# fims9000/SYNT_ISIC

Hardware: AMD Instinct MI355X
Metric: images/sec at 3x64x64 T=1000 (DDPM reverse-diffusion sampling) (higher is better)
Workload: dtype f32

## Files before the change

include/sisic.h:

```cpp
#ifndef SISIC_H
#define SISIC_H

#include <stdint.h>

#ifdef __cplusplus
extern "C" {
#endif

#define SISIC_ABI_VERSION 3

#define SISIC_OK 0
#define SISIC_EINVAL (-1)
#define SISIC_EHIP (-2)
#define SISIC_ESTATE (-3)
#define SISIC_ECANCEL (-4)

typedef struct sisic_ctx sisic_ctx;
typedef struct sisic_unet sisic_unet;
typedef struct sisic_resnet sisic_resnet;

int sisic_abi_version(void);
const char* sisic_last_error(void);

int sisic_create(int device_id, sisic_ctx** out);
int sisic_destroy(sisic_ctx* ctx);


typedef struct sisic_conv_args {
    const float* in0;
    const float* in1;
    int c0, c1;
    int B, Hin, Win;
    int upsample;
    int ksize;
    int stride;
    const float* w_packed;
    const float* bias;
    int Cout;
    const float* gn_scale;
    const float* gn_shift;
    int gn_silu;
    const float* chan_bias;
    int chan_bias_stride;
    const float* residual;
    int relu;
    float* out;
    int tile_cfg;
    const float* w_winograd;
    float* stats_out;
    const float* fin_gamma;
    const float* fin_beta;
    int fin_groups;
    float fin_eps;
    float* fin_scale;
    float* fin_shift;
    float* fin_mean_rstd;
} sisic_conv_args;

int sisic_conv_finalizes(const sisic_conv_args* args);

int sisic_conv_stats_slots(const sisic_conv_args* args);

int64_t sisic_conv_winograd_numel(int Cout, int Cin);
int sisic_conv_winograd_pack(sisic_ctx*, const float* w_oihw, int Cout, int Cin, float* u_packed, void* stream);

int64_t sisic_conv_s2_numel(int Cout, int Cin);
int sisic_conv_s2_pack(sisic_ctx*, const float* w_oihw, int Cout, int Cin, float* out, void* stream);

int64_t sisic_conv_packed_numel(int Cout, int Cin, int ksize);
int sisic_conv_pack_weights(sisic_ctx*, const float* w_oihw, int Cout, int Cin, int ksize,
                            float* w_packed, void* stream);
int sisic_conv2d(sisic_ctx*, const sisic_conv_args* args, void* stream);

int sisic_groupnorm_stats(sisic_ctx*, const float* in0, int c0, const float* in1, int c1,
                          int B, int HW, int groups, float eps,
                          const float* gamma, const float* beta,
                          float* scale, float* shift, void* stream);

int sisic_groupnorm_finalize(sisic_ctx*, const float* stats0, int c0, int slots0,
                             const float* stats1, int c1, int slots1,
                             int B, int HW, int groups, float eps,
                             const float* gamma, const float* beta,
                             float* scale, float* shift, void* stream);

int sisic_attention(sisic_ctx*, const float* qkv, float* out, int B, int C, int N, int head_dim,
                    void* stream);

int sisic_ddpm_step(sisic_ctx*, const float* eps, const float* x, const float* z, float* out,
                    int64_t n, float sqrt_beta_prod, float sqrt_alpha_prod, float c0, float c1,
                    float sigma, float clip, void* stream);

int sisic_denorm_u8(sisic_ctx*, const float* x, uint8_t* out, int B, int C, int H, int W, void* stream);
int sisic_denorm_u8_form(sisic_ctx*, const float* x, uint8_t* out, int B, int C, int H, int W, int form, void* stream);

typedef struct sisic_unet_config {
    int in_channels, out_channels;
    int layers_per_block;
    int n_blocks;
    int block_out_channels[8];
    int down_attn[8];
    int up_attn[8];
    int norm_groups;
    float norm_eps;
    int head_dim;
    int n_freqs;
    const float* freqs;
} sisic_unet_config;

int sisic_unet_create(sisic_ctx*, const sisic_unet_config* cfg, sisic_unet** out);
int sisic_unet_destroy(sisic_unet*);
int sisic_unet_num_tensors(const sisic_unet*);
const char* sisic_unet_tensor_name(const sisic_unet*, int index);
int sisic_unet_load(sisic_unet*, int n, const char* const* names, const float* const* host_ptrs,
                    const int64_t* numels);
int sisic_unet_set_latency_mode(sisic_unet*, int on);
int sisic_unet_set_graph_mode(sisic_unet*, int mode);
int64_t sisic_unet_graph_builds(const sisic_unet*);
int sisic_unet_forward(sisic_unet*, const float* sample, const int64_t* timesteps,
                       float* out, int B, int H, int W, void* stream);

int sisic_sample(sisic_unet*, float* x, int B, int H, int W, int T, const int64_t* timesteps,
                 const float* coef, float clip, const float* noise, float* traj, uint8_t* out_u8,
                 const volatile int* cancel, int* steps_done, void* stream);
int sisic_sample_frames(sisic_unet*, float* x, int B, int H, int W, int T, const int64_t* timesteps,
                        const float* coef, float clip, const float* noise, float* traj, const int* traj_row,
                        uint8_t* out_u8, const volatile int* cancel, int* steps_done, void* stream);

int sisic_noise_fill(sisic_ctx*, float* out, int B, int64_t n_per_image, const uint64_t* seeds, uint32_t step,
                     uint32_t tag, void* stream);
int sisic_noise_bits(sisic_ctx*, uint32_t* out, int B, int64_t n_per_image, const uint64_t* seeds, uint32_t step,
                     uint32_t tag, void* stream);
int sisic_ddpm_step_rng(sisic_ctx*, const float* eps, const float* x, float* out, int B, int64_t n_per_image,
                        const uint64_t* seeds_dev, uint32_t step, float sqrt_beta_prod, float sqrt_alpha_prod, float c0,
                        float c1, float sigma, float clip, void* stream);
int sisic_sample_frames_rng(sisic_unet*, float* x, int B, int H, int W, int T, const int64_t* timesteps,
                            const float* coef, float clip, const uint64_t* seeds, int step0, float* traj,
                            const int* traj_row, uint8_t* out_u8, const volatile int* cancel, int* steps_done,
                            void* stream);

int sisic_unet_train_begin(sisic_unet*);
int sisic_unet_train_end(sisic_unet*);
int sisic_add_noise(sisic_ctx*, const float* x0, const float* noise, const float* sqrt_alpha_prod,
                    const float* sqrt_one_minus_alpha_prod, float* out, int B, int64_t per_sample, void* stream);
int sisic_unet_train_forward(sisic_unet*, const float* sample, const int64_t* timesteps, float* out, int B, int H, int W,
                             void* stream);
int sisic_mse_loss(sisic_unet*, const float* pred, const float* target, int64_t n, float grad_scale, float* loss_dev,
                   float* dpred, void* stream);
int sisic_unet_backward(sisic_unet*, const float* dout, void* stream);
int sisic_unet_zero_grad(sisic_unet*, void* stream);
int sisic_unet_optimizer_step(sisic_unet*, double lr, double beta1, double beta2, double eps, float inv_scale, int* found_inf,
                              void* stream);
int sisic_unet_train_step(sisic_unet*, const float* images, const float* noise, const int64_t* timesteps,
                          const float* sqrt_alpha_prod, const float* sqrt_one_minus_alpha_prod, int B, int H, int W, double lr,
                          double beta1, double beta2, double eps, float loss_scale, float* loss_out, int* found_inf, void* stream);
int sisic_unet_read(sisic_unet*, int what, int index, float* host_out, int64_t numel);
int sisic_unet_write(sisic_unet*, int what, int index, const float* host_in, int64_t numel);
int64_t sisic_unet_train_steps(const sisic_unet*);

int sisic_conv2d_wgrad(sisic_ctx*, const sisic_conv_args* fwd_args, const float* dy, float* dw, void* stream);
int sisic_attention_bwd(sisic_ctx*, const float* qkv, const float* o, const float* dO, float* dqkv, int B, int C, int N,
                        int head_dim, void* stream);
int sisic_groupnorm_bwd(sisic_ctx*, const float* da, const float* x, int B, int C, int HW, int groups, float eps,
                        const float* gamma, const float* beta, int silu, float* dx_accum, float* dgamma, float* dbeta,
                        void* stream);

int sisic_resnet_create(sisic_ctx*, int num_classes, sisic_resnet** out);
int sisic_resnet_destroy(sisic_resnet*);
// ... 65 lines not shown
```

synt_isic_amd/_lib.py:

```python
from __future__ import annotations

import ctypes as C
import os
from typing import Optional

_LIB_PATH = os.environ.get("SISIC_LIB_PATH") or os.path.join(os.path.dirname(os.path.abspath(__file__)), "lib",
                                                             "libsisic_hip.so")
_lib: Optional[C.CDLL] = None

ABI_VERSION = 3

SISIC_OK = 0
SISIC_EINVAL = -1
SISIC_EHIP = -2
SISIC_ESTATE = -3
SISIC_ECANCEL = -4

c_float_p = C.POINTER(C.c_float)
c_int64_p = C.POINTER(C.c_int64)


class ConvArgs(C.Structure):
    _fields_ = [
        ("in0", C.c_void_p), ("in1", C.c_void_p),
        ("c0", C.c_int), ("c1", C.c_int),
        ("B", C.c_int), ("Hin", C.c_int), ("Win", C.c_int),
        ("upsample", C.c_int), ("ksize", C.c_int), ("stride", C.c_int),
        ("w_packed", C.c_void_p), ("bias", C.c_void_p), ("Cout", C.c_int),
        ("gn_scale", C.c_void_p), ("gn_shift", C.c_void_p), ("gn_silu", C.c_int),
        ("chan_bias", C.c_void_p), ("chan_bias_stride", C.c_int),
        ("residual", C.c_void_p), ("relu", C.c_int),
        ("out", C.c_void_p), ("tile_cfg", C.c_int),
        ("w_winograd", C.c_void_p),
        ("stats_out", C.c_void_p),
        ("fin_gamma", C.c_void_p), ("fin_beta", C.c_void_p), ("fin_groups", C.c_int), ("fin_eps", C.c_float),
        ("fin_scale", C.c_void_p), ("fin_shift", C.c_void_p), ("fin_mean_rstd", C.c_void_p),
    ]


class UNetConfigC(C.Structure):
    _fields_ = [
        ("in_channels", C.c_int), ("out_channels", C.c_int),
        ("layers_per_block", C.c_int), ("n_blocks", C.c_int),
        ("block_out_channels", C.c_int * 8),
        ("down_attn", C.c_int * 8), ("up_attn", C.c_int * 8),
        ("norm_groups", C.c_int), ("norm_eps", C.c_float), ("head_dim", C.c_int),
        ("n_freqs", C.c_int), ("freqs", c_float_p),
    ]


class InterventionJob(C.Structure):
    _fields_ = [("frame", C.c_int), ("mask", C.c_int), ("type", C.c_int), ("blur_kernel", C.c_int),
                ("noise_std", C.c_float)]


class AugmentParams(C.Structure):
    _fields_ = [("src", C.c_int32), ("crop_x", C.c_int32), ("crop_y", C.c_int32), ("crop_w", C.c_int32),
                ("crop_h", C.c_int32), ("hflip", C.c_int32), ("vflip", C.c_int32), ("order", C.c_int32 * 3),
                ("factor", C.c_float * 3), ("rotate", C.c_int32), ("rot", C.c_int32 * 6), ("reserved", C.c_int32 * 4)]


SIGNATURES = {
    "sisic_abi_version": (C.c_int, []),
    "sisic_last_error": (C.c_char_p, []),
    "sisic_create": (C.c_int, [C.c_int, C.POINTER(C.c_void_p)]),
    "sisic_destroy": (C.c_int, [C.c_void_p]),
    "sisic_conv_packed_numel": (C.c_int64, [C.c_int, C.c_int, C.c_int]),
    "sisic_conv_pack_weights": (C.c_int, [C.c_void_p, C.c_void_p, C.c_int, C.c_int, C.c_int, C.c_void_p, C.c_void_p]),
    "sisic_conv_winograd_numel": (C.c_int64, [C.c_int, C.c_int]),
    "sisic_conv_winograd_pack": (C.c_int, [C.c_void_p, C.c_void_p, C.c_int, C.c_int, C.c_void_p, C.c_void_p]),
    "sisic_conv_s2_numel": (C.c_int64, [C.c_int, C.c_int]),
    "sisic_conv_s2_pack": (C.c_int, [C.c_void_p, C.c_void_p, C.c_int, C.c_int, C.c_void_p, C.c_void_p]),
    "sisic_conv2d": (C.c_int, [C.c_void_p, C.POINTER(ConvArgs), C.c_void_p]),
    "sisic_conv_stats_slots": (C.c_int, [C.POINTER(ConvArgs)]),
    "sisic_conv_finalizes": (C.c_int, [C.POINTER(ConvArgs)]),
    "sisic_groupnorm_finalize": (C.c_int, [C.c_void_p, C.c_void_p, C.c_int, C.c_int, C.c_void_p, C.c_int, C.c_int,
                                           C.c_int, C.c_int, C.c_int, C.c_float, C.c_void_p, C.c_void_p, C.c_void_p,
                                           C.c_void_p, C.c_void_p]),
    "sisic_groupnorm_stats": (C.c_int, [C.c_void_p, C.c_void_p, C.c_int, C.c_void_p, C.c_int, C.c_int, C.c_int,
                                        C.c_int, C.c_float, C.c_void_p, C.c_void_p, C.c_void_p, C.c_void_p,
                                        C.c_void_p]),
    "sisic_attention": (C.c_int, [C.c_void_p, C.c_void_p, C.c_void_p, C.c_int, C.c_int, C.c_int, C.c_int, C.c_void_p]),
    "sisic_ddpm_step": (C.c_int, [C.c_void_p, C.c_void_p, C.c_void_p, C.c_void_p, C.c_void_p, C.c_int64,
                                  C.c_float, C.c_float, C.c_float, C.c_float, C.c_float, C.c_float, C.c_void_p]),
    "sisic_denorm_u8": (C.c_int, [C.c_void_p, C.c_void_p, C.c_void_p, C.c_int, C.c_int, C.c_int, C.c_int, C.c_void_p]),
    "sisic_denorm_u8_form": (C.c_int, [C.c_void_p, C.c_void_p, C.c_void_p, C.c_int, C.c_int, C.c_int, C.c_int, C.c_int,
                                       C.c_void_p]),
    "sisic_unet_create": (C.c_int, [C.c_void_p, C.POINTER(UNetConfigC), C.POINTER(C.c_void_p)]),
    "sisic_unet_destroy": (C.c_int, [C.c_void_p]),
    "sisic_unet_num_tensors": (C.c_int, [C.c_void_p]),
    "sisic_unet_tensor_name": (C.c_char_p, [C.c_void_p, C.c_int]),
    "sisic_unet_load": (C.c_int, [C.c_void_p, C.c_int, C.POINTER(C.c_char_p), C.POINTER(C.c_void_p), c_int64_p]),
    "sisic_unet_set_latency_mode": (C.c_int, [C.c_void_p, C.c_int]),
    "sisic_unet_set_graph_mode": (C.c_int, [C.c_void_p, C.c_int]),
    "sisic_unet_graph_builds": (C.c_int64, [C.c_void_p]),
    "sisic_unet_forward": (C.c_int, [C.c_void_p, C.c_void_p, c_int64_p, C.c_void_p, C.c_int, C.c_int, C.c_int,
                                     C.c_void_p]),
    "sisic_sample": (C.c_int, [C.c_void_p, C.c_void_p, C.c_int, C.c_int, C.c_int, C.c_int, c_int64_p, c_float_p,
                               C.c_float, C.c_void_p, C.c_void_p, C.c_void_p, C.POINTER(C.c_int), C.POINTER(C.c_int),
                               C.c_void_p]),
    "sisic_sample_frames": (C.c_int, [C.c_void_p, C.c_void_p, C.c_int, C.c_int, C.c_int, C.c_int, c_int64_p, c_float_p,
                                      C.c_float, C.c_void_p, C.c_void_p, C.POINTER(C.c_int), C.c_void_p, C.POINTER(C.c_int),
                                      C.POINTER(C.c_int), C.c_void_p]),
    "sisic_noise_fill": (C.c_int, [C.c_void_p, C.c_void_p, C.c_int, C.c_int64, C.POINTER(C.c_uint64), C.c_uint32,
                                   C.c_uint32, C.c_void_p]),
    "sisic_noise_bits": (C.c_int, [C.c_void_p, C.c_void_p, C.c_int, C.c_int64, C.POINTER(C.c_uint64), C.c_uint32,
                                   C.c_uint32, C.c_void_p]),
    "sisic_ddpm_step_rng": (C.c_int, [C.c_void_p, C.c_void_p, C.c_void_p, C.c_void_p, C.c_int, C.c_int64, C.c_void_p,
                                      C.c_uint32, C.c_float, C.c_float, C.c_float, C.c_float, C.c_float, C.c_float,
                                      C.c_void_p]),
    "sisic_sample_frames_rng": (C.c_int, [C.c_void_p, C.c_void_p, C.c_int, C.c_int, C.c_int, C.c_int, c_int64_p, c_float_p,
                                          C.c_float, C.POINTER(C.c_uint64), C.c_int, C.c_void_p, C.POINTER(C.c_int),
                                          C.c_void_p, C.POINTER(C.c_int), C.POINTER(C.c_int), C.c_void_p]),
    "sisic_unet_train_begin": (C.c_int, [C.c_void_p]),
    "sisic_unet_train_end": (C.c_int, [C.c_void_p]),
    "sisic_add_noise": (C.c_int, [C.c_void_p, C.c_void_p, C.c_void_p, C.c_void_p, C.c_void_p, C.c_void_p, C.c_int,
                                  C.c_int64, C.c_void_p]),
    "sisic_unet_train_forward": (C.c_int, [C.c_void_p, C.c_void_p, c_int64_p, C.c_void_p, C.c_int, C.c_int, C.c_int,
                                           C.c_void_p]),
    "sisic_mse_loss": (C.c_int, [C.c_void_p, C.c_void_p, C.c_void_p, C.c_int64, C.c_float, C.c_void_p, C.c_void_p,
                                 C.c_void_p]),
    "sisic_unet_backward": (C.c_int, [C.c_void_p, C.c_void_p, C.c_void_p]),
    "sisic_unet_zero_grad": (C.c_int, [C.c_void_p, C.c_void_p]),
    "sisic_unet_optimizer_step": (C.c_int, [C.c_void_p, C.c_double, C.c_double, C.c_double, C.c_double, C.c_float,
                                            C.POINTER(C.c_int), C.c_void_p]),
    "sisic_unet_train_step": (C.c_int, [C.c_void_p, C.c_void_p, C.c_void_p, c_int64_p, c_float_p, c_float_p, C.c_int,
                                        C.c_int, C.c_int, C.c_double, C.c_double, C.c_double, C.c_double, C.c_float,
                                        C.POINTER(C.c_float), C.POINTER(C.c_int), C.c_void_p]),
    "sisic_unet_read": (C.c_int, [C.c_void_p, C.c_int, C.c_int, c_float_p, C.c_int64]),
    "sisic_unet_write": (C.c_int, [C.c_void_p, C.c_int, C.c_int, c_float_p, C.c_int64]),
    "sisic_unet_train_steps": (C.c_int64, [C.c_void_p]),
    "sisic_conv2d_wgrad": (C.c_int, [C.c_void_p, C.POINTER(ConvArgs), C.c_void_p, C.c_void_p, C.c_void_p]),
    "sisic_attention_bwd": (C.c_int, [C.c_void_p, C.c_void_p, C.c_void_p, C.c_void_p, C.c_void_p, C.c_int, C.c_int, C.c_int,
                                      C.c_int, C.c_void_p]),
    "sisic_groupnorm_bwd": (C.c_int, [C.c_void_p, C.c_void_p, C.c_void_p, C.c_int, C.c_int, C.c_int, C.c_int, C.c_float,
                                      C.c_void_p, C.c_void_p, C.c_int, C.c_void_p, C.c_void_p, C.c_void_p, C.c_void_p]),
    "sisic_resnet_create": (C.c_int, [C.c_void_p, C.c_int, C.POINTER(C.c_void_p)]),
    "sisic_resnet_destroy": (C.c_int, [C.c_void_p]),
    "sisic_resnet_num_tensors": (C.c_int, [C.c_void_p]),
    "sisic_resnet_tensor_name": (C.c_char_p, [C.c_void_p, C.c_int]),
    "sisic_resnet_load": (C.c_int, [C.c_void_p, C.c_int, C.POINTER(C.c_char_p), C.POINTER(C.c_void_p), c_int64_p]),
    "sisic_resnet_randomize": (C.c_int, [C.c_void_p, C.c_uint64, C.c_uint32, C.c_float, C.c_void_p]),
    "sisic_resnet_restore": (C.c_int, [C.c_void_p, C.c_void_p]),
    "sisic_resnet_forward": (C.c_int, [C.c_void_p, C.c_void_p, C.c_void_p, C.c_int, C.c_int, C.c_int, C.c_int,
                                       C.c_void_p]),
    "sisic_resnet_stem": (C.c_int, [C.c_void_p, C.c_void_p, C.c_void_p, C.c_int, C.c_int, C.c_int, C.c_int, C.c_void_p]),
    "sisic_resnet_input_gradient": (C.c_int, [C.c_void_p, C.c_void_p, C.c_int, C.c_int, C.c_int, C.c_int, C.c_void_p,
                                              C.c_void_p, C.c_void_p]),
    "sisic_resnet_gradcam": (C.c_int, [C.c_void_p, C.c_void_p, C.c_int, C.c_int, C.c_int, C.c_int, C.c_void_p,
                                       C.c_void_p, C.c_void_p]),
    "sisic_resnet_workspace_bytes": (C.c_int64, [C.c_void_p]),
    "sisic_unet_workspace_bytes": (C.c_int64, [C.c_void_p]),
    "sisic_class_scores": (C.c_int, [C.c_void_p, C.c_void_p, C.c_int, C.c_int, C.c_int, C.c_void_p, C.c_void_p,
                                     C.c_void_p]),
    "sisic_mask_patches": (C.c_int, [C.c_void_p, C.c_void_p, C.c_void_p, C.c_void_p, C.c_int, C.c_int, C.c_int,
                                     C.c_int, C.c_int, C.c_void_p]),
    "sisic_intervene": (C.c_int, [C.c_void_p, C.c_void_p, C.c_int, C.c_void_p, C.c_int, C.c_int, C.c_int, C.c_int, C.c_int,
                                  C.POINTER(InterventionJob), C.POINTER(C.c_uint64), C.c_void_p, C.c_void_p, C.c_void_p,
                                  C.c_void_p, C.c_void_p]),
    "sisic_cfi_metrics": (C.c_int, [C.c_void_p, C.c_void_p, C.c_int, C.c_void_p, C.c_int, C.c_int, C.POINTER(C.c_int),
                                    C.c_void_p, C.c_void_p]),
# ... 48 lines not shown
```

synt_isic_amd/csrc/api.cpp:

```cpp
#include <cstring>

#include "common.h"

namespace sisic {

static thread_local char g_err[1024] = "";

void set_error(const char* fmt, ...) {
    va_list ap;
    va_start(ap, fmt);
    vsnprintf(g_err, sizeof(g_err), fmt, ap);
    va_end(ap);
}

static hipEvent_t take_event(sisic_ctx* ctx) {
    if (!ctx->event_pool.empty()) {
        hipEvent_t e = ctx->event_pool.back();
        ctx->event_pool.pop_back();
        return e;
    }
    hipEvent_t e = nullptr;
    if (hipEventCreate(&e) != hipSuccess) return nullptr;
    return e;
}

ProfileScope::ProfileScope(sisic_ctx* c, hipStream_t s, int kind, double bytes, double flops, double flops_exec, int kind2)
    : ctx(c), stream(s) {
    if (!c || !c->profiling) return;
    ev.start = take_event(c);
    ev.stop = take_event(c);
    ev.kind = kind;
    ev.kind2 = kind2;
    if (!ev.start || !ev.stop) return;
    for (int k : {kind, kind2}) {
        if (k < 0) continue;
        c->prof[k].bytes += bytes;
        c->prof[k].flops += flops;
        c->prof[k].flops_exec += (flops_exec < 0.0) ? flops : flops_exec;
        c->prof[k].launches += 1;
    }
    (void)hipEventRecord(ev.start, s);
    active = true;
}

ProfileScope::~ProfileScope() {
    if (!active) return;
    (void)hipEventRecord(ev.stop, stream);
    ctx->pending.push_back(ev);
}

int profile_collect(sisic_ctx* ctx) {
    for (auto& ev : ctx->pending) {
        SISIC_HIP(hipEventSynchronize(ev.stop));
        float ms = 0.f;
        SISIC_HIP(hipEventElapsedTime(&ms, ev.start, ev.stop));
        ctx->prof[ev.kind].ms += ms;
        if (ev.kind2 >= 0) ctx->prof[ev.kind2].ms += ms;
        ctx->event_pool.push_back(ev.start);
        ctx->event_pool.push_back(ev.stop);
    }
    ctx->pending.clear();
    return SISIC_OK;
}

}

using namespace sisic;

extern "C" {

int sisic_abi_version(void) { return SISIC_ABI_VERSION; }

const char* sisic_last_error(void) { return sisic::g_err; }

int sisic_create(int device_id, sisic_ctx** out) {
    SISIC_REQUIRE(out != nullptr, "sisic_create: out is NULL");
    *out = nullptr;
    int n = 0;
    SISIC_HIP(hipGetDeviceCount(&n));
    SISIC_REQUIRE(device_id >= 0 && device_id < n, "sisic_create: device %d of %d", device_id, n);
    SISIC_HIP(hipSetDevice(device_id));
    hipDeviceProp_t prop;
    SISIC_HIP(hipGetDeviceProperties(&prop, device_id));
    SISIC_REQUIRE(std::strncmp(prop.gcnArchName, "gfx950", 6) == 0,
                  "sisic_create: device %d is %s; this library is built for gfx950 (MI355X) only", device_id,
                  prop.gcnArchName);
    auto* ctx = new sisic_ctx();
    ctx->device = device_id;
    ctx->num_cus = prop.multiProcessorCount;
    *out = ctx;
    return SISIC_OK;
}

int sisic_destroy(sisic_ctx* ctx) {
    if (!ctx) return SISIC_OK;
    (void)profile_collect(ctx);
    for (auto e : ctx->event_pool) (void)hipEventDestroy(e);
    for (auto& kv : ctx->splitk)
        if (kv.second.p) (void)hipFree(kv.second.p);
    for (auto& it : ctx->bf3_items) {
        if (it.fill_done) (void)hipEventDestroy(it.fill_done);
        if (it.tab) (void)hipFree(it.tab);
    }
    delete ctx;
    return SISIC_OK;
}

int64_t sisic_conv_packed_numel(int Cout, int Cin, int ksize) {
    if (Cout <= 0 || Cin <= 0 || (ksize != 1 && ksize != 3 && ksize != 7)) return -1;
    return conv_packed_floats(Cout, Cin, ksize);
}

int sisic_conv_pack_weights(sisic_ctx* ctx, const float* w, int Cout, int Cin, int ksize, float* packed, void* stream) {
    SISIC_REQUIRE(ctx && w && packed && Cout > 0 && Cin > 0, "conv_pack_weights: bad arguments");
    return launch_conv_pack(ctx, w, Cout, Cin, ksize, packed, static_cast<hipStream_t>(stream));
}

int64_t sisic_conv_s2_numel(int Cout, int Cin) {
    if (Cout <= 0 || Cin <= 0) return -1;
    return conv_s2_packed_floats(Cout, Cin);
}

int sisic_conv_s2_pack(sisic_ctx* ctx, const float* w, int Cout, int Cin, float* out, void* stream) {
    SISIC_REQUIRE(ctx && w && out && Cout > 0 && Cin > 0, "conv_s2_pack: bad arguments");
    return launch_conv_s2_pack(ctx, w, Cout, Cin, out, static_cast<hipStream_t>(stream));
}

int64_t sisic_conv_winograd_numel(int Cout, int Cin) {
    if (Cout <= 0 || Cin <= 0) return -1;
    return winograd_packed_numel(Cout, Cin);
}

int sisic_conv_winograd_pack(sisic_ctx* ctx, const float* w, int Cout, int Cin, float* packed, void* stream) {
    SISIC_REQUIRE(ctx && w && packed && Cout > 0 && Cin > 0, "conv_winograd_pack: bad arguments");
    return launch_winograd_pack(ctx, w, Cout, Cin, packed, static_cast<hipStream_t>(stream));
}

int sisic_conv2d(sisic_ctx* ctx, const sisic_conv_args* args, void* stream) {
    SISIC_REQUIRE(ctx && args, "conv2d: null argument");
    return launch_conv2d(ctx, *args, static_cast<hipStream_t>(stream));
}

int sisic_conv_stats_slots(const sisic_conv_args* args) { return args ? conv_stats_slots(*args) : 0; }
int sisic_conv_finalizes(const sisic_conv_args* args) { return args && conv_finalizes(*args) ? 1 : 0; }

int sisic_groupnorm_finalize(sisic_ctx* ctx, const float* stats0, int c0, int slots0, const float* stats1, int c1,
                             int slots1, int B, int HW, int groups, float eps, const float* gamma, const float* beta,
                             float* scale, float* shift, void* stream) {
    SISIC_REQUIRE(ctx, "groupnorm_finalize: null context");
    return launch_gn_finalize(ctx, stats0, c0, slots0, stats1, c1, slots1, B, HW, groups, eps, gamma, beta, scale,
                              shift, static_cast<hipStream_t>(stream));
}

int sisic_groupnorm_stats(sisic_ctx* ctx, const float* in0, int c0, const float* in1, int c1, int B, int HW,
                          int groups, float eps, const float* gamma, const float* beta, float* scale, float* shift,
                          void* stream) {
    SISIC_REQUIRE(ctx, "groupnorm_stats: null context");
    return launch_gn_stats(ctx, in0, c0, in1, c1, B, HW, groups, eps, gamma, beta, scale, shift,
                           static_cast<hipStream_t>(stream));
}

int sisic_attention(sisic_ctx* ctx, const float* qkv, float* out, int B, int C, int N, int head_dim, void* stream) {
    SISIC_REQUIRE(ctx, "attention: null context");
    return launch_attention(ctx, qkv, out, B, C, N, head_dim, static_cast<hipStream_t>(stream));
}

int sisic_ddpm_step(sisic_ctx* ctx, const float* eps, const float* x, const float* z, float* out, int64_t n,
                    float sqrt_beta_prod, float sqrt_alpha_prod, float c0, float c1, float sigma, float clip,
                    void* stream) {
    SISIC_REQUIRE(ctx, "ddpm_step: null context");
    return launch_ddpm_step(ctx, eps, x, z, out, n, sqrt_beta_prod, sqrt_alpha_prod, c0, c1, sigma, clip,
                            static_cast<hipStream_t>(stream));
}

int sisic_noise_fill(sisic_ctx* ctx, float* out, int B, int64_t n_per_image, const uint64_t* seeds, uint32_t step,
                     uint32_t tag, void* stream) {
    SISIC_REQUIRE(ctx, "noise_fill: null context");
    return launch_noise_fill(ctx, out, B, n_per_image, seeds, step, tag, false, static_cast<hipStream_t>(stream));
}

int sisic_noise_bits(sisic_ctx* ctx, uint32_t* out, int B, int64_t n_per_image, const uint64_t* seeds, uint32_t step,
                     uint32_t tag, void* stream) {
    SISIC_REQUIRE(ctx, "noise_bits: null context");
    return launch_noise_fill(ctx, out, B, n_per_image, seeds, step, tag, true, static_cast<hipStream_t>(stream));
}

int sisic_ddpm_step_rng(sisic_ctx* ctx, const float* eps, const float* x, float* out, int B, int64_t n_per_image,
                        const uint64_t* seeds_dev, uint32_t step, float sqrt_beta_prod, float sqrt_alpha_prod, float c0,
                        float c1, float sigma, float clip, void* stream) {
    SISIC_REQUIRE(ctx && B > 0 && n_per_image > 0, "ddpm_step_rng: null context or empty batch");
    return launch_ddpm_step_rng(ctx, eps, x, out, (int64_t)B * n_per_image, n_per_image, seeds_dev, step, sqrt_beta_prod,
                                sqrt_alpha_prod, c0, c1, sigma, clip, static_cast<hipStream_t>(stream));
}

int sisic_denorm_u8(sisic_ctx* ctx, const float* x, uint8_t* out, int B, int C, int H, int W, void* stream) {
    SISIC_REQUIRE(ctx, "denorm_u8: null context");
    return launch_denorm_u8(ctx, x, out, B, C, H, W, static_cast<hipStream_t>(stream));
}

int sisic_denorm_u8_form(sisic_ctx* ctx, const float* x, uint8_t* out, int B, int C, int H, int W, int form, void* stream) {
    SISIC_REQUIRE(ctx, "denorm_u8_form: null context");
    return launch_denorm_u8(ctx, x, out, B, C, H, W, static_cast<hipStream_t>(stream), form);
}

int sisic_intervene(sisic_ctx* ctx, const float* frames, int F, const uint8_t* masks, int M, int C, int H, int W, int J,
                    const sisic_intervention_job* jobs, const uint64_t* seeds, const int32_t* src_index, float* out,
                    float* intervention_out, float* stats, void* stream) {
    SISIC_REQUIRE(ctx, "intervene: null context");
    return launch_intervene(ctx, frames, F, masks, M, C, H, W, J, jobs, seeds, src_index, out, intervention_out, stats,
                            static_cast<hipStream_t>(stream));
}

int sisic_cfi_metrics(sisic_ctx* ctx, const float* logits_orig, int F, const float* logits_mod, int J, int n_classes,
                      const int* job_frame, float* rows, void* stream) {
    SISIC_REQUIRE(ctx, "cfi_metrics: null context");
    return launch_cfi_metrics(ctx, logits_orig, F, logits_mod, J, n_classes, job_frame, rows, static_cast<hipStream_t>(stream));
}

int sisic_resample_diffs(sisic_ctx* ctx, const double* top, int n_top, const double* bottom, int n_bottom, uint64_t seed,
                         int n_bootstrap, int n_permutations, double* boot_out, double* perm_out, void* stream) {
    SISIC_REQUIRE(ctx, "resample_diffs: null context");
    return launch_resample_diffs(ctx, top, n_top, bottom, n_bottom, seed, n_bootstrap, n_permutations, boot_out, perm_out,
                                 static_cast<hipStream_t>(stream));
}

int sisic_augment(sisic_ctx* ctx, const uint8_t* dataset, int N, int H, int W, const sisic_augment_params* params_dev, int B,
                  int32_t* gray_mean_scratch, float* out, void* stream) {
    SISIC_REQUIRE(ctx, "augment: null context");
    return launch_augment(ctx, dataset, N, H, W, params_dev, B, gray_mean_scratch, out, false, static_cast<hipStream_t>(stream));
}

int sisic_augment_u8(sisic_ctx* ctx, const uint8_t* dataset, int N, int H, int W, const sisic_augment_params* params_dev,
                     int B, int32_t* gray_mean_scratch, uint8_t* out_hwc, void* stream) {
    SISIC_REQUIRE(ctx, "augment_u8: null context");
    return launch_augment(ctx, dataset, N, H, W, params_dev, B, gray_mean_scratch, out_hwc, true, static_cast<hipStream_t>(stream));
}
// ... 28 lines not shown
```

synt_isic_amd/csrc/common.h:

```cpp
#pragma once

#include <hip/hip_runtime.h>

#include <atomic>
#include <cstdarg>
#include <cstdint>
#include <cstdio>
#include <string>
#include <map>
#include <mutex>
#include <vector>

#include "../../include/sisic.h"

namespace sisic {

void set_error(const char* fmt, ...);

#define SISIC_HIP(call)                                                                   \
    do {                                                                                  \
        hipError_t _e = (call);                                                           \
        if (_e != hipSuccess) {                                                           \
            ::sisic::set_error("%s failed: %s (%s:%d)", #call, hipGetErrorString(_e),     \
                               __FILE__, __LINE__);                                       \
// ... 9 lines not shown
        }                                        \
    } while (0)

#define SISIC_TRY(expr)             \
    do {                            \
        int _rc = (expr);           \
        if (_rc != SISIC_OK) return _rc; \
    } while (0)

enum ProfileKind { PK_CONV3 = 0, PK_CONV1 = 1, PK_GN = 2, PK_ATTN = 3, PK_DDPM = 4, PK_OTHER = 5, PK_WINO_MAIN = 6, PK_WINO_BF3 = 7, PK_COUNT = 8 };

struct ProfileSlot {
    double ms = 0, bytes = 0, flops = 0, flops_exec = 0;
    int64_t launches = 0;
};

struct PendingEvent {
    hipEvent_t start, stop;
    int kind;
    int kind2;
};

}

struct sisic_ctx {
    int device = 0;
    int num_cus = 0;
    bool profiling = false;
    sisic::ProfileSlot prof[sisic::PK_COUNT];
    std::vector<sisic::PendingEvent> pending;
    std::vector<hipEvent_t> event_pool;
    struct SplitK { float* p = nullptr; size_t floats = 0; };
    std::map<hipStream_t, SplitK> splitk;
    std::mutex splitk_mutex;
    struct Bf3Items { int key[9]; unsigned* tab = nullptr; hipStream_t fill_stream = nullptr; hipEvent_t fill_done = nullptr; };
    std::vector<Bf3Items> bf3_items;
    std::mutex bf3_items_mutex;
    std::atomic<uint64_t> scratch_generation{0};
};

namespace sisic {

struct ProfileScope {
    sisic_ctx* ctx;
    hipStream_t stream;
    PendingEvent ev{};
    bool active = false;
    ProfileScope(sisic_ctx* c, hipStream_t s, int kind, double bytes, double flops, double flops_exec = -1.0, int kind2 = -1);
    ~ProfileScope();
};

int profile_collect(sisic_ctx* ctx);

inline int ensure_dynamic_lds(sisic_ctx* ctx, const void* kern, int bytes, std::atomic<uint64_t>& done) {
    const uint64_t bit = uint64_t(1) << (ctx->device & 63);
    if (done.load(std::memory_order_acquire) & bit) return SISIC_OK;
    SISIC_HIP(hipFuncSetAttribute(kern, hipFuncAttributeMaxDynamicSharedMemorySize, bytes));
    done.fetch_or(bit, std::memory_order_release);
    return SISIC_OK;
}

inline int cdiv(int a, int b) { return (a + b - 1) / b; }
inline int wino_latency_ksplit(int Cout, int Cin, int Hout, int Wout) {
    const int co_t = Cout > 64 ? 128 : 64;
    const int per_image = cdiv(Hout, 8) * cdiv(Wout, 16) * cdiv(Cout, co_t);
    const int nchunks = cdiv(Cin, 8);
    int k = 1;
    while (per_image * k < 256 && k < 8 && nchunks % (2 * k) == 0) k *= 2;
    return k;
}
inline int wino_latency_segments(int Hout, int Wout) { return cdiv(Hout * Wout, 1024); }
inline int64_t cdiv64(int64_t a, int64_t b) { return (a + b - 1) / b; }
inline int round_up(int a, int b) { return cdiv(a, b) * b; }

constexpr int CONV_CO_TILE = 64;
inline int conv_ci_chunk(int ksize) { return ksize == 1 ? 32 : (ksize == 3 ? 16 : 4); }
inline int conv_cin_pad(int cin, int ksize) { return round_up(cin, conv_ci_chunk(ksize)); }
inline int conv_cout_pad(int cout) { return round_up(cout, CONV_CO_TILE); }
inline int64_t conv_packed_floats(int cout, int cin, int ksize) {
    const int64_t first = (int64_t)conv_cin_pad(cin, ksize) * ksize * ksize * conv_cout_pad(cout);
    return ksize == 1 ? 3 * first + first / 2 : first;
}

int launch_conv2d(sisic_ctx*, const sisic_conv_args& a, hipStream_t s);
int launch_conv_smallcout(sisic_ctx*, const sisic_conv_args& a, hipStream_t s);
int launch_score_head_bwd(sisic_ctx*, const float* logits, const float* fc_w, const float* act, float* g, int B, int C,
                          int HW, int n_classes, int target, hipStream_t s);
int launch_relu_bwd(sisic_ctx*, const float* dy, const float* y, float* out, int64_t n, hipStream_t s);
int launch_scatter_add_even(sisic_ctx*, float* dst, const float* src, int planes, int H, int W, hipStream_t s);
int launch_maxpool_bwd(sisic_ctx*, const float* dm, const float* xin, float* dx, int planes, int H, int W, hipStream_t s);
int launch_stem_bwd(sisic_ctx*, const float* g, const float* w_oihw, float* dp, int B, int CO, int OH, int OW, int H, int W,
                    hipStream_t s);
int launch_preprocess_bwd(sisic_ctx*, const float* dp, const float* x, float* dx, int B, int H, int W, int OH, int OW,
                          hipStream_t s);
int launch_add_relu(sisic_ctx*, const float* y, const float* identity, float* out, int64_t n, hipStream_t s);
int launch_gradcam(sisic_ctx*, const float* y, const float* outp, const float* fc_w, const float* bias, float* cam, int B, int C,
                   int h, int w, int S, int target, hipStream_t s);
int conv_stats_slots(const sisic_conv_args& a);
bool conv_finalizes(const sisic_conv_args& a);
bool conv_pointwise_applicable(const sisic_conv_args& a);
int conv_pointwise_stats_slots(const sisic_conv_args& a);
int launch_conv_pointwise(sisic_ctx*, const sisic_conv_args& a, hipStream_t s);
bool conv_pointwise_bf3_applicable(const sisic_conv_args& a);
int launch_conv_pointwise_bf3(sisic_ctx*, const sisic_conv_args& a, hipStream_t s);
bool conv_s2_bf3_applicable(const sisic_conv_args& a);
int conv_s2_bf3_stats_slots(const sisic_conv_args& a);
int launch_conv_s2_bf3(sisic_ctx*, const sisic_conv_args& a, hipStream_t s);
int64_t conv_s2_packed_floats(int Cout, int Cin);
int launch_conv_s2_pack(sisic_ctx*, const float* w, int Cout, int Cin, float* out, hipStream_t s);
int launch_gn_finalize(sisic_ctx*, const float* st0, int c0, int slots0, const float* st1, int c1, int slots1, int B,
                       int HW, int groups, float eps, const float* gamma, const float* beta, float* scale, float* shift,
                       hipStream_t s, float* mean_rstd = nullptr);
int launch_conv_winograd(sisic_ctx*, const sisic_conv_args& a, const float* u_packed, int cfg, hipStream_t s);
int launch_winograd_pack(sisic_ctx*, const float* w, int Cout, int Cin, float* packed, hipStream_t s);
int64_t winograd_packed_numel(int Cout, int Cin);
inline int64_t winograd_first_floats(int Cout, int Cin) { return (int64_t)round_up(Cin, 16) * 16 * conv_cout_pad(Cout); }
int launch_conv_pack(sisic_ctx*, const float* w, int Cout, int Cin, int k, float* packed, hipStream_t s);
int launch_gn_stats(sisic_ctx*, const float* in0, int c0, const float* in1, int c1, int B, int HW, int groups,
                    float eps, const float* gamma, const float* beta, float* scale, float* shift, hipStream_t s,
                    float* mean_rstd = nullptr);
int launch_attention(sisic_ctx*, const float* qkv, float* out, int B, int C, int N, int head_dim, hipStream_t s);
int launch_ddpm_step(sisic_ctx*, const float* eps, const float* x, const float* z, float* out, int64_t n,
                     float sb, float sa, float c0, float c1, float sigma, float clip, hipStream_t s);
size_t loop_state_bytes();
int launch_loop_select_row(sisic_ctx*, const float* table, int R, const void* state, float* out, hipStream_t s);
int launch_loop_advance(sisic_ctx*, void* state, hipStream_t s);
int launch_ddpm_step_indexed(sisic_ctx*, const float* eps, float* x, int64_t n, const void* state, const float* coef,
                             const int* zrow, float clip, hipStream_t s);
int launch_ddpm_step_rng(sisic_ctx*, const float* eps, const float* x, float* out, int64_t n, int64_t n_per_image,
                         const uint64_t* seeds_dev, uint32_t step, float sb, float sa, float c0, float c1, float sigma,
                         float clip, hipStream_t s);
int launch_ddpm_step_indexed_rng(sisic_ctx*, const float* eps, float* x, int64_t n, int64_t n_per_image, const void* state,
                                 const float* coef, const uint64_t* seeds_dev, float clip, hipStream_t s);
int launch_noise_fill(sisic_ctx*, void* out, int B, int64_t n_per_image, const uint64_t* seeds_host, uint32_t step,
                      uint32_t tag, bool bits, hipStream_t s);
int launch_denorm_u8(sisic_ctx*, const float* x, uint8_t* out, int B, int C, int H, int W, hipStream_t s, int form = 0);
int launch_temb_mlp(sisic_ctx*, const float* t_vals, int B, const float* freqs, int n_freqs, const float* w1t,
                    const float* b1, const float* w2t, const float* b2, int hidden, float* temb_act, hipStream_t s,
                    float* save_emb = nullptr, float* save_h1 = nullptr, float* save_t2 = nullptr);
int launch_linear_t(sisic_ctx*, const float* x, int B, int K, const float* wt, const float* bias, int R,
                    float* out, hipStream_t s);
int launch_transpose2d(sisic_ctx*, const float* in, int rows, int cols, float* out, int out_ld, int out_col0,
                       hipStream_t s);
int launch_preprocess(sisic_ctx*, const float* x, float* out, int B, int H, int W, int OH, int OW, hipStream_t s);
int launch_maxpool(sisic_ctx*, const float* x, float* out, int B, int C, int H, int W, hipStream_t s);
int launch_avgpool_fc(sisic_ctx*, const float* x, const float* w, const float* bias, float* out, int B, int C, int HW,
                      int n_out, hipStream_t s);
int launch_class_scores(sisic_ctx*, const float* logits, int B, int n, int target, float* prob, float* logscore,
                        hipStream_t s);
int launch_mask_patches(sisic_ctx*, const float* image, const uint8_t* masks, float* out, int S, int C, int H, int W,
                        int patch, hipStream_t s);

int launch_intervene(sisic_ctx*, const float* frames, int F, const uint8_t* masks, int M, int C, int H, int W, int J,
                     const sisic_intervention_job* jobs, const uint64_t* seeds, const int32_t* src_index, float* out,
                     float* intervention_out, float* stats, hipStream_t s);
int launch_cfi_metrics(sisic_ctx*, const float* logits_orig, int F, const float* logits_mod, int J, int n,
                       const int* job_frame, float* rows, hipStream_t s);
int launch_resample_diffs(sisic_ctx*, const double* top, int n_top, const double* bottom, int n_bottom, uint64_t seed,
                          int n_bootstrap, int n_permutations, double* boot_out, double* perm_out, hipStream_t s);
int launch_randomize_weight(sisic_ctx*, float* raw, float* raw_t, const double* sc, int cout, int cin, int k, uint64_t seed,
                            uint32_t trial, uint32_t tag, float strength, hipStream_t s);

int launch_augment(sisic_ctx*, const uint8_t* dataset, int N, int H, int W, const sisic_augment_params* params_dev, int B,
                   int32_t* gray_mean_scratch, void* out, bool u8, hipStream_t s);

}
```

synt_isic_amd/csrc/conv_mfma.hip:

```cpp
#include <cstdlib>
#include <type_traits>

#include "common.h"
#include "pack_device.h"

namespace sisic {

typedef float f32x16 __attribute__((ext_vector_type(16)));

struct ConvParams {
    const float* in0;
    const float* in1;
    int c0, c1;
    int B, Hin, Win;
    int Hc, Wc;
    int Hout, Wout;
    int ups;
    int zero_insert;
    const float* w;
    int cout_pad;
    const float* bias;
    int Cout;
    const float* gn_scale;
    const float* gn_shift;
// ... 322 lines not shown
                psum[m][r] += pv ? v : 0.0f;
            }
        }
    }

    if (p.stats) {
        const float cnt = half_wave_sum((float)__builtin_popcount(pvmask));
        const float inv = 1.0f / fmaxf(cnt, 1.0f);
        const int slots = p.tiles_x * p.tiles_y * WN, slot = (ty * p.tiles_x + tx) * WN + wn;
#pragma unroll
        for (int m = 0; m < MT; ++m) {
#pragma unroll
            for (int r = 0; r < 16; ++r) {
                const int co = co0 + wm * MT * 32 + m * 32 + (r & 3) + 8 * (r >> 2) + 4 * half;
                const float s1 = half_wave_sum(psum[m][r]);
                const float mean = s1 * inv;
                float q = 0.0f;
#pragma unroll
                for (int n = 0; n < NT; ++n) {
                    const float d = acc[m][n][r] - mean;
                    q += ((pvmask >> n) & 1u) ? d * d : 0.0f;
                }
                q = half_wave_sum(q);
                if (l31 == 0 && co < p.Cout)
                    reinterpret_cast<float4*>(p.stats)[((size_t)b * p.Cout + co) * slots + slot] = make_float4(cnt, s1, q, 0.0f);
            }
        }
    }
}


__global__ void conv_pack_kernel(const float* __restrict__ w, int Cout, int Cin, int KK, int cin_pad, int cout_pad,
                                 float* __restrict__ out) {
    const size_t first = (size_t)cin_pad * KK * cout_pad;
    const size_t total = KK == 1 ? 3 * first + first / 2 : first;
    for (size_t i = (size_t)blockIdx.x * blockDim.x + threadIdx.x; i < total; i += (size_t)gridDim.x * blockDim.x) {
        conv_pack_elem(i, w, Cout, Cin, KK, cin_pad, cout_pad, out);
    }
}

template <int KS, int STRIDE, int MT, int NT, int WM, int WN, int TW, int CIC, int OCC = 2, int KSP = 1>
static int launch_cfg(sisic_ctx* ctx, ConvParams& p, hipStream_t s) {
    using G = ConvGeom<KS, STRIDE, MT, NT, WM, WN, TW, CIC, KSP>;
    p.tiles_x = cdiv(p.Wout, TW);
    p.tiles_y = cdiv(p.Hout, G::TH);
    p.n_co_tiles = p.cout_pad / G::CO_TILE;
    p.nchunks = cdiv(p.c0 + p.c1, CIC);
    const int64_t nwg = (int64_t)p.B * p.tiles_x * p.tiles_y * p.n_co_tiles;
    SISIC_REQUIRE(nwg > 0 && nwg < (int64_t(1) << 31), "conv2d: grid of %lld workgroups unsupported", (long long)nwg);
    p.nwg = (int)nwg;
    if (p.slots_query) {
        *p.slots_query = p.tiles_x * p.tiles_y * WN;
        return SISIC_OK;
    }
    if constexpr (KS == 1 && STRIDE == 1 && TW == G::PIX && G::EPT % 4 == 0) {
        const bool aligned = ((reinterpret_cast<uintptr_t>(p.in0) | reinterpret_cast<uintptr_t>(p.in1)) & 15) == 0;
        if (p.Wc % 4 == 0 && aligned) {
            auto kern4 = conv_mfma_kernel<KS, STRIDE, MT, NT, WM, WN, TW, CIC, OCC, KSP, true>;
            static std::atomic<uint64_t> lds_opt_in4{0};
            SISIC_TRY(ensure_dynamic_lds(ctx, reinterpret_cast<const void*>(kern4), (int)G::LDS_BYTES, lds_opt_in4));
            hipLaunchKernelGGL(kern4, dim3(p.nwg), dim3(G::NTHR), G::LDS_BYTES, s, p);
            SISIC_HIP(hipGetLastError());
            return SISIC_OK;
        }
    }
    auto kern = conv_mfma_kernel<KS, STRIDE, MT, NT, WM, WN, TW, CIC, OCC, KSP>;
    static std::atomic<uint64_t> lds_opt_in{0};
    SISIC_TRY(ensure_dynamic_lds(ctx, reinterpret_cast<const void*>(kern), (int)G::LDS_BYTES, lds_opt_in));
    hipLaunchKernelGGL(kern, dim3(p.nwg), dim3(G::NTHR), G::LDS_BYTES, s, p);
    SISIC_HIP(hipGetLastError());
    return SISIC_OK;
}

int launch_conv_pack(sisic_ctx*, const float* w, int Cout, int Cin, int k, float* packed, hipStream_t s) {
    SISIC_REQUIRE(k == 1 || k == 3 || k == 7, "conv_pack: ksize %d unsupported", k);
    const int cin_pad = conv_cin_pad(Cin, k), cout_pad = conv_cout_pad(Cout);
    const size_t total = (size_t)cin_pad * k * k * cout_pad;
    const int blocks = (int)std::min<size_t>((total * (k == 1 ? 4 : 1) + 255) / 256, 4096);
    hipLaunchKernelGGL(conv_pack_kernel, dim3(blocks), dim3(256), 0, s, w, Cout, Cin, k * k, cin_pad, cout_pad, packed);
    SISIC_HIP(hipGetLastError());
    return SISIC_OK;
}

static int dispatch_conv2d(sisic_ctx* ctx, const sisic_conv_args& a, hipStream_t s, int* slots_query);

static int winograd_cfg(const sisic_conv_args& a) {
    if (!(a.ksize == 3 && a.stride == 1 && a.w_winograd != nullptr && a.Cout > 4) || a.upsample == 2) return 0;
    if ((a.tile_cfg >= 60 && a.tile_cfg <= 74) || a.tile_cfg == 78 || a.tile_cfg == 79 || (a.tile_cfg >= 90 && a.tile_cfg <= 92)) return a.tile_cfg;
    if (a.tile_cfg != 0) return 0;
    const int Hout = a.Hin << (a.upsample ? 1 : 0), Wout = a.Win << (a.upsample ? 1 : 0);
    const bool fits32 = 16.0 * std::max(a.c0, a.c1) * a.Hin * a.Win < 4294967296.0;
    if (!fits32) return 0;
    if (Hout >= 12 && Wout >= 12) {
        static const bool wide_on = [] { const char* e = std::getenv("SISIC_WINO_WIDE"); return !e || std::atoi(e) != 0; }();
        static const bool bf3_on = [] { const char* e = std::getenv("SISIC_WINO_BF16X3"); return !e || std::atoi(e) != 0; }();
        const int th = (Hout + 15) / 16 * 16, tw = (Wout + 15) / 16 * 16;
        if (bf3_on && a.Cout % 64 == 0 && 4 * Hout * Wout >= 3 * th * tw && a.c0 + a.c1 >= 16 &&
            a.c0 + a.c1 <= 2048 &&
            4.0 * a.Cout * Hout * Wout < 2147483648.0)
            return 74;
        if (wide_on && !a.upsample) return a.Cout > 64 ? 68 : 69;
        return 66;
    }
    const int Cin = a.c0 + a.c1;
    static const bool ksplit_on = [] { const char* e = std::getenv("SISIC_KSPLIT"); return !e || std::atoi(e) != 0; }();
    if (ksplit_on && Hout <= 8 && Wout <= 8 && Hout >= 5 && Wout >= 5 && Cin >= 128 && Cin % 32 == 0 && a.Cout >= 128) {
        static const bool wide_on = [] { const char* e = std::getenv("SISIC_WINO_WIDE"); return !e || std::atoi(e) != 0; }();
        static const bool bf3_on = [] { const char* e = std::getenv("SISIC_WINO_BF16X3"); return !e || std::atoi(e) != 0; }();
        if (bf3_on && !a.upsample && a.Cout % 64 == 0 && Cin <= 512) return 92;
        return (wide_on && !a.upsample) ? 91 : 90;
    }
    return 0;
}
static bool winograd_selected(const sisic_conv_args& a) { return winograd_cfg(a) != 0; }

int conv_stats_slots(const sisic_conv_args& a) {
    if (const int cfg = winograd_cfg(a)) {
        if (cfg >= 90 && cfg <= 92) return 1;
        const int Hout = a.Hin << (a.upsample ? 1 : 0), Wout = a.Win << (a.upsample ? 1 : 0);
        if ((cfg == 78 || cfg == 79) && wino_latency_ksplit(a.Cout, a.c0 + a.c1, Hout, Wout) > 1) return wino_latency_segments(Hout, Wout);
        if ((cfg >= 68 && cfg <= 73) || cfg == 78 || cfg == 79) return ((Hout + 7) / 8) * ((Wout + 15) / 16);
        const int edge = (cfg == 61 || cfg == 63 || cfg == 65 || cfg == 67) ? 8 : 16;
        return ((Hout + edge - 1) / edge) * ((Wout + edge - 1) / edge);
    }
    int slots = 0;
    sisic_conv_args q = a;
    q.stats_out = nullptr;
    if (dispatch_conv2d(nullptr, q, nullptr, &slots) != SISIC_OK) return 0;
    return slots;
}

bool conv_finalizes(const sisic_conv_args& a) {
    if (!a.fin_gamma || a.fin_groups <= 0) return false;
    const int cfg = winograd_cfg(a);
    const int Hout = a.Hin << (a.upsample ? 1 : 0), Wout = a.Win << (a.upsample ? 1 : 0);
    if (a.Cout % a.fin_groups != 0 || a.Cout / a.fin_groups != 8) return false;
    if (cfg == 74) return !a.upsample && Hout <= 16 && Wout <= 16 && a.Cout % 64 == 0;
    if (cfg < 90 || cfg > 92) return false;
    if (Hout * Wout != 64 || a.Cout % 16 != 0) return false;
    return ((reinterpret_cast<uintptr_t>(a.residual) | reinterpret_cast<uintptr_t>(a.out) | reinterpret_cast<uintptr_t>(a.stats_out)) & 15) == 0;
}

int launch_conv2d(sisic_ctx* ctx, const sisic_conv_args& a, hipStream_t s) { return dispatch_conv2d(ctx, a, s, nullptr); }

static int dispatch_conv2d(sisic_ctx* ctx, const sisic_conv_args& a, hipStream_t s, int* slots_query) {
    SISIC_REQUIRE(a.in0 && a.w_packed && a.out, "conv2d: null tensor");
    SISIC_REQUIRE(a.B > 0 && a.Hin > 0 && a.Win > 0 && a.c0 > 0 && a.c1 >= 0 && a.Cout > 0, "conv2d: bad shape");
    SISIC_REQUIRE((a.c1 == 0) == (a.in1 == nullptr), "conv2d: in1/c1 mismatch");
    SISIC_REQUIRE(a.ksize == 1 || a.ksize == 3 || a.ksize == 7, "conv2d: ksize %d unsupported", a.ksize);
    SISIC_REQUIRE(a.stride == 1 || a.stride == 2, "conv2d: stride %d unsupported", a.stride);
    SISIC_REQUIRE(a.ksize != 7 || a.stride == 2, "conv2d: 7x7 is built for stride 2 only (the ResNet stem)");
    SISIC_REQUIRE(!(a.upsample && a.stride != 1), "conv2d: upsample with stride");
    SISIC_REQUIRE((a.gn_scale == nullptr) == (a.gn_shift == nullptr), "conv2d: gn_scale/gn_shift mismatch");

    ConvParams p{};
    p.in0 = a.in0; p.in1 = a.in1; p.c0 = a.c0; p.c1 = a.c1;
    p.B = a.B; p.Hin = a.Hin; p.Win = a.Win;
    p.ups = a.upsample ? 1 : 0;
    p.zero_insert = a.upsample == 2 ? 1 : 0;
    p.Hc = a.Hin << p.ups; p.Wc = a.Win << p.ups;
    const int pad = a.ksize / 2;
    p.Hout = (p.Hc + 2 * pad - a.ksize) / a.stride + 1;
    p.Wout = (p.Wc + 2 * pad - a.ksize) / a.stride + 1;
    p.w = a.w_packed; p.cout_pad = conv_cout_pad(a.Cout);
    p.bias = a.bias; p.Cout = a.Cout;
    p.gn_scale = a.gn_scale; p.gn_shift = a.gn_shift; p.gn_silu = a.gn_silu;
    p.chan_bias = a.chan_bias; p.chan_bias_stride = a.chan_bias_stride; p.residual = a.residual; p.relu = a.relu; p.out = a.out;
    p.stats = a.stats_out; p.slots_query = slots_query;

    const int Cin = a.c0 + a.c1;
    const double kk = double(a.ksize) * a.ksize;
    const double out_elems = double(a.B) * a.Cout * p.Hout * p.Wout;
    const double bytes = 4.0 * (double(a.B) * Cin * a.Hin * a.Win + out_elems) + 4.0 * (Cin * a.Cout * kk + a.Cout) +
                         (a.residual ? 4.0 * out_elems : 0.0);
    const double flops = 2.0 * out_elems * Cin * kk;
    int cfg = a.tile_cfg;
    const bool use_wino = winograd_selected(a);
    SISIC_REQUIRE(a.stats_out == nullptr || conv_stats_slots(a) > 0,
                  "conv2d: stats_out given but sisic_conv_stats_slots() is 0 for these arguments");
    const bool wino_ups9 = use_wino && a.upsample && !a.gn_scale && winograd_cfg(a) == 66;
    ProfileScope prof(slots_query ? nullptr : ctx, s, a.ksize == 1 ? PK_CONV1 : PK_CONV3, bytes, flops,
                      use_wino ? flops * (wino_ups9 ? 9.0 : 16.0) / 36.0 : flops,
                      (use_wino && winograd_cfg(a) == 74) ? PK_WINO_BF3 :
                      (use_wino && !wino_ups9 && (winograd_cfg(a) == 66 || (winograd_cfg(a) >= 68 && winograd_cfg(a) <= 73) || winograd_cfg(a) == 78 || winograd_cfg(a) == 79)) ? PK_WINO_MAIN : -1);

    if (a.ksize == 3 && a.stride == 1 && !a.upsample && a.Cout <= 4 && (cfg == 0 || (cfg >= 50 && cfg <= 52))) {
        if (slots_query) return SISIC_OK;
        return launch_conv_smallcout(ctx, a, s);
    }
    if (use_wino) {
        SISIC_REQUIRE(!slots_query, "conv2d: internal: slot query on the Winograd path");
        return launch_conv_winograd(ctx, a, a.w_winograd, winograd_cfg(a), s);
    }
    SISIC_REQUIRE((cfg < 60 || cfg > 74) && cfg != 78 && cfg != 79 && (cfg < 90 || cfg > 92), "conv2d: tile_cfg %d needs w_winograd, ksize 3 and stride 1", cfg);
    if (a.ksize == 7) {
        if (cfg == 0) cfg = 41;
        if (cfg == 41) return launch_cfg<7, 2, 2, 1, 1, 4, 32, 2>(ctx, p, s);
        if (cfg == 42) return launch_cfg<7, 2, 2, 1, 1, 4, 32, 4>(ctx, p, s);
    } else if (a.ksize == 1 && a.stride == 2) {
        if (cfg == 0) cfg = p.Wout >= 24 ? 31 : (p.Wout >= 12 ? 32 : 33);
        switch (cfg) {
            case 31: return launch_cfg<1, 2, 2, 1, 1, 4, 32, 16>(ctx, p, s);
            case 32: return launch_cfg<1, 2, 2, 1, 1, 4, 16, 16>(ctx, p, s);
            case 33: return launch_cfg<1, 2, 1, 1, 2, 2, 8, 16>(ctx, p, s);
        }
    } else if (a.ksize == 1) {
        p.Hin = 1; p.Win = a.Hin * a.Win; p.Hc = 1; p.Wc = p.Win; p.Hout = 1; p.Wout = p.Win; p.ups = 0;
        SISIC_REQUIRE(!a.upsample, "conv2d: 1x1 with upsample");
        static const bool pw_on = [] { const char* e = std::getenv("SISIC_POINTWISE"); return !e || std::atoi(e) != 0; }();
        static const bool pwb_on = [] { const char* e = std::getenv("SISIC_POINTWISE_BF16X3"); return !e || std::atoi(e) != 0; }();
        if ((cfg == 0 && pwb_on && conv_pointwise_bf3_applicable(a)) || (cfg >= 28 && cfg <= 30) || cfg == 34 || cfg == 35) {
            if (slots_query) { *slots_query = conv_pointwise_stats_slots(a); return SISIC_OK; }
            return launch_conv_pointwise_bf3(ctx, a, s);
        }
        if ((cfg == 0 && pw_on && conv_pointwise_applicable(a)) || cfg == 20) {
            if (slots_query) { *slots_query = conv_pointwise_stats_slots(a); return SISIC_OK; }
            return launch_conv_pointwise(ctx, a, s);
        }
        if (cfg == 0) cfg = (p.Wout <= 64) ? 22 : (p.Wout <= 256 ? 25 : 24);
        switch (cfg) {
            case 21: return launch_cfg<1, 1, 2, 2, 1, 4, 256, 16>(ctx, p, s);
            case 22: return launch_cfg<1, 1, 1, 1, 2, 2, 64, 16>(ctx, p, s);
            case 23: return launch_cfg<1, 1, 2, 1, 1, 4, 128, 16>(ctx, p, s);
            case 24: return launch_cfg<1, 1, 1, 2, 2, 4, 256, 32, 4>(ctx, p, s);
            case 25: return launch_cfg<1, 1, 1, 1, 2, 4, 128, 32, 4>(ctx, p, s);
            case 26: return launch_cfg<1, 1, 1, 2, 2, 4, 256, 16, 4>(ctx, p, s);
            case 27: return launch_cfg<1, 1, 1, 1, 2, 4, 128, 16, 4>(ctx, p, s);
        }
    } else if (a.stride == 1) {
        if (cfg == 0) cfg = p.Wout >= 24 ? 8 : (p.Wout >= 12 ? 9 : 16);
        switch (cfg) {
            case 1: return launch_cfg<3, 1, 2, 2, 1, 4, 64, 8>(ctx, p, s);
            case 2: return launch_cfg<3, 1, 2, 2, 1, 4, 32, 8>(ctx, p, s);
            case 3: return launch_cfg<3, 1, 2, 2, 1, 4, 16, 8>(ctx, p, s);
            case 4: return launch_cfg<3, 1, 1, 1, 2, 2, 8, 8>(ctx, p, s);
            case 16: return launch_cfg<3, 1, 1, 1, 2, 2, 8, 16, 2, 2>(ctx, p, s);
            case 17: return launch_cfg<3, 1, 1, 1, 2, 2, 8, 8, 2, 2>(ctx, p, s);
            case 5: return launch_cfg<3, 1, 2, 1, 1, 4, 16, 8>(ctx, p, s);
            case 6: return launch_cfg<3, 1, 2, 1, 1, 4, 64, 8>(ctx, p, s);
            case 7: return launch_cfg<3, 1, 2, 1, 1, 4, 32, 8>(ctx, p, s);
            case 8: return launch_cfg<3, 1, 1, 2, 2, 4, 32, 8, 4>(ctx, p, s);
            case 9: return launch_cfg<3, 1, 1, 2, 2, 4, 16, 8, 4>(ctx, p, s);
            case 10: return launch_cfg<3, 1, 1, 2, 2, 4, 32, 8, 2>(ctx, p, s);
            case 14: return launch_cfg<3, 1, 1, 1, 2, 4, 16, 8, 4>(ctx, p, s);
            case 15: return launch_cfg<3, 1, 1, 1, 2, 4, 8, 8, 4>(ctx, p, s);
        }
    } else {
        static const bool s2b_on = [] { const char* e = std::getenv("SISIC_S2_BF16X3"); return !e || std::atoi(e) != 0; }();
        if ((cfg == 0 && s2b_on && conv_s2_bf3_applicable(a)) || cfg == 36) {
            if (slots_query) { *slots_query = conv_s2_bf3_applicable(a) ? conv_s2_bf3_stats_slots(a) : 0; return SISIC_OK; }
            return launch_conv_s2_bf3(ctx, a, s);
        }
        if (cfg == 0) cfg = p.Wout >= 24 ? 11 : (p.Wout >= 12 ? 12 : 18);
        switch (cfg) {
            case 11: return launch_cfg<3, 2, 2, 1, 1, 4, 32, 8>(ctx, p, s);
            case 12: return launch_cfg<3, 2, 2, 1, 1, 4, 16, 8>(ctx, p, s);
            case 13: return launch_cfg<3, 2, 1, 1, 2, 2, 8, 8>(ctx, p, s);
            case 18: return launch_cfg<3, 2, 1, 1, 2, 2, 8, 16, 2, 2>(ctx, p, s);
            case 19: return launch_cfg<3, 2, 1, 1, 2, 2, 8, 8, 2, 2>(ctx, p, s);
        }
    }
    set_error("conv2d: tile_cfg %d invalid for ksize %d stride %d", cfg, a.ksize, a.stride);
    return SISIC_EINVAL;
}

}
```

synt_isic_amd/csrc/conv_pointwise_bf3.hip:

```cpp
#include <cstdlib>
#include <type_traits>

#include "common.h"

namespace sisic {

typedef float pwb_f32x16 __attribute__((ext_vector_type(16)));
typedef short pwb_bf16x8 __attribute__((ext_vector_type(8)));
typedef unsigned pwb_u4 __attribute__((ext_vector_type(4)));
typedef unsigned pwb_u2 __attribute__((ext_vector_type(2)));
typedef float pwb_f2 __attribute__((ext_vector_type(2)));
typedef float pwb_f4 __attribute__((ext_vector_type(4)));

struct PwbParams {
    const float* in0;
    const float* in1;
    int c0, c1, B, HW;
    const float* wb;
    int n_co64;
    const float* bias;
    int Cout;
    const float* gn_scale;
    const float* gn_shift;
    const float* chan_bias;
    int chan_bias_stride;
    const float* residual;
    int relu;
    float* out;
    float* stats;
    int n_px, n_co_items, nitems, nwg, nchunks;
};

constexpr int PWB_WAVES = 4;

__device__ __forceinline__ float pwb_half_wave_sum(float v) {
    v += __int_as_float(__builtin_amdgcn_update_dpp(0, __float_as_int(v), 0xB1, 0xf, 0xf, true));
    v += __int_as_float(__builtin_amdgcn_update_dpp(0, __float_as_int(v), 0x4E, 0xf, 0xf, true));
    v += __int_as_float(__builtin_amdgcn_update_dpp(0, __float_as_int(v), 0x141, 0xf, 0xf, true));
    v += __int_as_float(__builtin_amdgcn_update_dpp(0, __float_as_int(v), 0x140, 0xf, 0xf, true));
    return v + __shfl_xor(v, 16);
}
__device__ __forceinline__ float pwb_row16_sum(float v) {
    v += __int_as_float(__builtin_amdgcn_update_dpp(0, __float_as_int(v), 0xB1, 0xf, 0xf, true));
    v += __int_as_float(__builtin_amdgcn_update_dpp(0, __float_as_int(v), 0x4E, 0xf, 0xf, true));
    v += __int_as_float(__builtin_amdgcn_update_dpp(0, __float_as_int(v), 0x141, 0xf, 0xf, true));
    v += __int_as_float(__builtin_amdgcn_update_dpp(0, __float_as_int(v), 0x140, 0xf, 0xf, true));
    return v;
}
__device__ __forceinline__ float pwb_silu(float v) { return v * __builtin_amdgcn_rcpf(1.0f + __expf(-v)); }

template <int PRO, int NB>
__global__ void __launch_bounds__(64 * PWB_WAVES, 4) conv_pwb_kernel(const PwbParams p) {
    extern __shared__ __attribute__((aligned(16))) float smem[];
    int wg;
    {
        const int L = blockIdx.x, nwg = p.nwg;
        const int xcd = L & 7, slot = L >> 3, q = nwg >> 3, r = nwg & 7;
        wg = (xcd < r ? xcd * (q + 1) : r * (q + 1) + (xcd - r) * q) + slot;
    }
    const int tid = threadIdx.x, lane = tid & 63;
    const int wave_u = __builtin_amdgcn_readfirstlane(tid >> 6);
    const int item = wg * PWB_WAVES + wave_u;
    if (item >= p.nitems) return;
    const int half = lane >> 5, l31 = lane & 31;
    int co_i = item % p.n_co_items;
    const int t = item / p.n_co_items;
    int px_t = t % p.n_px, b = t / p.n_px;
    asm volatile("" : "+s"(co_i), "+s"(px_t), "+s"(b));
    constexpr int CB = 2;
    const int px0 = 32 * NB * px_t, co0 = 64 * co_i;
    const int Cin = p.c0 + p.c1, HW = p.HW, n = p.nchunks;

    const __amdgpu_buffer_rsrc_t rs0 = __builtin_amdgcn_make_buffer_rsrc(const_cast<float*>(p.in0 + (size_t)b * p.c0 * HW), 0, -1, 0x00020000);
    const __amdgpu_buffer_rsrc_t rs1 = __builtin_amdgcn_make_buffer_rsrc(
        const_cast<float*>(p.in1 ? p.in1 + (size_t)b * p.c1 * HW : p.in0), 0, -1, 0x00020000);
    const __amdgpu_buffer_rsrc_t rsw = __builtin_amdgcn_make_buffer_rsrc(const_cast<float*>(p.wb), 0, -1, 0x00020000);

    const unsigned x_voff = 4u * (unsigned)((4 * half) * HW + px0 + NB * l31);
    const unsigned a_lane16 = 16u * (unsigned)lane, a_lane8 = 8u * (unsigned)lane;

    float* const gnL = smem + wave_u * (2 * Cin);
    if constexpr (PRO != 0) {
        for (int i = lane; i < Cin; i += 64) {
            gnL[2 * i] = p.gn_scale[(size_t)b * Cin + i];
            gnL[2 * i + 1] = p.gn_shift[(size_t)b * Cin + i];
        }
        asm volatile("s_waitcnt lgkmcnt(0)" ::: "memory");
        __builtin_amdgcn_wave_barrier();
    }

    pwb_f32x16 acc[CB][NB];
#pragma unroll
    for (int x = 0; x < CB; ++x)
#pragma unroll
        for (int nb = 0; nb < NB; ++nb)
#pragma unroll
            for (int r = 0; r < 16; ++r) acc[x][nb][r] = 0.0f;

    struct XRegs {
        pwb_f2 x[4];
    };
    auto ld = [&](const __amdgpu_buffer_rsrc_t rs, unsigned soff) {
        if constexpr (NB == 2) return __builtin_bit_cast(pwb_f2, __builtin_amdgcn_raw_buffer_load_b64(rs, x_voff, soff, 0));
        else return pwb_f2{__builtin_bit_cast(float, __builtin_amdgcn_raw_buffer_load_b32(rs, x_voff, soff, 0)), 0.0f};
    };
    pwb_u4 ua[CB];
    pwb_u2 ul[CB];
    pwb_u4 ub[CB];
    pwb_u2 um[CB];
    auto load_x = [&](int c, XRegs& r) {
#ifdef PWB_DIAG_NO_X_LOADS
        if (c > 1) return;
#endif
        const int cc0 = 8 * c;
        if (cc0 < p.c0) {
            const unsigned soff = 4u * (unsigned)(cc0 * HW);
#pragma unroll
            for (int k = 0; k < 4; ++k)
                r.x[k] = ld(rs0, soff + 4u * (unsigned)(k * HW));
        } else {
            const unsigned soff = 4u * (unsigned)((cc0 - p.c0) * HW);
#pragma unroll
            for (int k = 0; k < 4; ++k)
                r.x[k] = ld(rs1, soff + 4u * (unsigned)(k * HW));
        }
    };
    auto load_a = [&](int c) {
#ifdef PWB_DIAG_NO_FILTER_LOADS
        if (c > 1) return;
#endif
        const unsigned s0 = 3072u * (unsigned)(c * p.n_co64 + co_i);
#pragma unroll
        for (int x = 0; x < CB; ++x) {
            ua[x] = __builtin_amdgcn_raw_buffer_load_b128(rsw, a_lane16, s0 + 1024u * (unsigned)x, 0);
            ul[x] = __builtin_amdgcn_raw_buffer_load_b64(rsw, a_lane8, s0 + 2048u + 512u * (unsigned)x, 0);
        }
    };
    auto load_b = [&](int c) {
#ifdef PWB_DIAG_NO_FILTER_LOADS
// ... 88 lines not shown
            Tup u = make(c + 1, rb, 0);
            mm_with(t, Z{}, ua, ul);
            weave();
            load_a(c + 2);
            if (c + 3 < n) load_x(c + 3, rb);
            t = make(c + 2, ra, 0);
            mm_with(u, Z{}, ub, um);
            weave();
            if (c + 3 < n) load_b(c + 3);
        }
        if (c + 1 < n) {
            Tup u = make(c + 1, rb, 0);
            mm_with(t, Z{}, ua, ul);
            mm_with(u, Z{}, ub, um);
        } else {
            mm_with(t, Z{}, ua, ul);
        }
    }

    const __amdgpu_buffer_rsrc_t rso = __builtin_amdgcn_make_buffer_rsrc(p.out + (size_t)b * p.Cout * HW, 0, -1, 0x00020000);
    const __amdgpu_buffer_rsrc_t rsr = __builtin_amdgcn_make_buffer_rsrc(
        const_cast<float*>(p.residual ? p.residual + (size_t)b * p.Cout * HW : p.out), 0, -1, 0x00020000);
    const unsigned o_voff = 4u * (unsigned)((4 * half) * HW + px0 + NB * l31);
    const int slots = HW / 32;
#pragma unroll
    for (int x = 0; x < CB; ++x) {
        float add[16];
        pwb_f2 res[16];
#pragma unroll
        for (int r = 0; r < 16; ++r) {
            const int cs = co0 + 32 * x + 8 * (r >> 2) + (r & 3);
            const int col = cs + 4 * half;
            add[r] = 0.0f;
            if (p.bias) add[r] += p.bias[col];
            if (p.chan_bias) add[r] += p.chan_bias[(size_t)b * p.chan_bias_stride + col];
            res[r] = pwb_f2{0.0f, 0.0f};
            if (p.residual) {
                if constexpr (NB == 2) res[r] = __builtin_bit_cast(pwb_f2, __builtin_amdgcn_raw_buffer_load_b64(rsr, o_voff, 4u * (unsigned)(cs * HW), 0));
                else res[r].x = __builtin_bit_cast(float, __builtin_amdgcn_raw_buffer_load_b32(rsr, o_voff, 4u * (unsigned)(cs * HW), 0));
            }
        }
#pragma unroll
        for (int r = 0; r < 16; ++r) {
            const int cs = co0 + 32 * x + 8 * (r >> 2) + (r & 3);
            float vv[2] = {0.0f, 0.0f};
#pragma unroll
            for (int nb = 0; nb < NB; ++nb) {
                vv[nb] = acc[x][nb][r] + add[r] + (nb ? res[r].y : res[r].x);
                if (p.relu) vv[nb] = fmaxf(vv[nb], 0.0f);
            }
            if constexpr (NB == 2) __builtin_amdgcn_raw_buffer_store_b64(pwb_u2{__float_as_uint(vv[0]), __float_as_uint(vv[1])}, rso, o_voff, 4u * (unsigned)(cs * HW), 0);
            else __builtin_amdgcn_raw_buffer_store_b32(__float_as_uint(vv[0]), rso, o_voff, 4u * (unsigned)(cs * HW), 0);
            if (p.stats) {
                const int co = cs + 4 * half;
                if constexpr (NB == 1) {
                    const float s1 = pwb_half_wave_sum(vv[0]);
                    const float d = vv[0] - s1 * (1.0f / 32.0f);
                    float dd;
                    asm volatile("v_mul_f32 %0, %1, %1" : "=v"(dd) : "v"(d));
                    const float q = pwb_half_wave_sum(dd);
                    if (l31 == 0)
                        reinterpret_cast<float4*>(p.stats)[((size_t)b * p.Cout + co) * slots + px_t] = make_float4(32.0f, s1, q, 0.0f);
                } else {
                    const float s1 = pwb_row16_sum(vv[0] + vv[1]);
                    const float mean = s1 * (1.0f / 32.0f);
                    const float d0 = vv[0] - mean, d1 = vv[1] - mean;
                    float q0, q1;
                    asm volatile("v_mul_f32 %0, %2, %2\n\tv_mul_f32 %1, %3, %3" : "=&v"(q0), "=&v"(q1) : "v"(d0), "v"(d1));
                    const float q = pwb_row16_sum(q0 + q1);
                    if ((l31 & 15) == 0)
                        reinterpret_cast<float4*>(p.stats)[((size_t)b * p.Cout + co) * slots + 2 * px_t + (l31 >> 4)] = make_float4(32.0f, s1, q, 0.0f);
                }
            }
        }
    }
}

#ifndef PWBK_VAR
#define PWBK_VAR 0
#endif
template <int PRO>
__global__ void __launch_bounds__(64 * PWB_WAVES, 4) conv_pwbk_kernel(const PwbParams p) {
    extern __shared__ __attribute__((aligned(16))) float smem[];
    int item;
    {
        const int L = blockIdx.x, nwg = p.nwg;
        const int xcd = L & 7, slot = L >> 3, q = nwg >> 3, r = nwg & 7;
        item = (xcd < r ? xcd * (q + 1) : r * (q + 1) + (xcd - r) * q) + slot;
    }
    const int tid = threadIdx.x, lane = tid & 63;
    const int wave_u = __builtin_amdgcn_readfirstlane(tid >> 6);
    const int half = lane >> 5, l31 = lane & 31;
    int co_i = item % p.n_co_items;
    const int t = item / p.n_co_items;
    int px_t = t % p.n_px, b = t / p.n_px;
    asm volatile("" : "+s"(co_i), "+s"(px_t), "+s"(b));
    constexpr int CB = 2;
    const int px0 = 32 * px_t, co0 = 64 * co_i;
    const int Cin = p.c0 + p.c1, HW = p.HW;
    const int nl = p.nchunks / PWB_WAVES, cb = wave_u * nl;

    const __amdgpu_buffer_rsrc_t rs0 = __builtin_amdgcn_make_buffer_rsrc(const_cast<float*>(p.in0 + (size_t)b * p.c0 * HW), 0, -1, 0x00020000);
    const __amdgpu_buffer_rsrc_t rs1 = __builtin_amdgcn_make_buffer_rsrc(
        const_cast<float*>(p.in1 ? p.in1 + (size_t)b * p.c1 * HW : p.in0), 0, -1, 0x00020000);
    const __amdgpu_buffer_rsrc_t rsw = __builtin_amdgcn_make_buffer_rsrc(const_cast<float*>(p.wb), 0, -1, 0x00020000);
    const unsigned x_voff = 4u * (unsigned)((4 * half) * HW + px0 + l31);
    const unsigned a_lane16 = 16u * (unsigned)lane, a_lane8 = 8u * (unsigned)lane;

    float* const P_lds = smem;
    float* const gnL = smem + PWB_WAVES * 32 * 64 + wave_u * (2 * 8 * nl);
    if constexpr (PRO != 0) {
        for (int i = lane; i < 8 * nl; i += 64) {
            gnL[2 * i] = p.gn_scale[(size_t)b * Cin + 8 * cb + i];
            gnL[2 * i + 1] = p.gn_shift[(size_t)b * Cin + 8 * cb + i];
        }
        asm volatile("s_waitcnt lgkmcnt(0)" ::: "memory");
        __builtin_amdgcn_wave_barrier();
    }

    pwb_f32x16 acc[CB];
#pragma unroll
    for (int x = 0; x < CB; ++x)
#pragma unroll
        for (int r = 0; r < 16; ++r) acc[x][r] = 0.0f;
    struct XRegs { float x[4]; };
    auto load_x = [&](int c, XRegs& r) {
        const int cc0 = 8 * c;
        if (cc0 < p.c0) {
            const unsigned soff = 4u * (unsigned)(cc0 * HW);
#pragma unroll
            for (int k = 0; k < 4; ++k) r.x[k] = __builtin_bit_cast(float, __builtin_amdgcn_raw_buffer_load_b32(rs0, x_voff, soff + 4u * (unsigned)(k * HW), 0));
        } else {
            const unsigned soff = 4u * (unsigned)((cc0 - p.c0) * HW);
#pragma unroll
            for (int k = 0; k < 4; ++k) r.x[k] = __builtin_bit_cast(float, __builtin_amdgcn_raw_buffer_load_b32(rs1, x_voff, soff + 4u * (unsigned)(k * HW), 0));
        }
    };
    auto load_f = [&](int c, pwb_u4 (&fa)[CB], pwb_u2 (&fl)[CB]) {
        const unsigned s0 = 3072u * (unsigned)(c * p.n_co64 + co_i);
#pragma unroll
        for (int x = 0; x < CB; ++x) {
            fa[x] = __builtin_amdgcn_raw_buffer_load_b128(rsw, a_lane16, s0 + 1024u * (unsigned)x, 0);
#if (PWBK_VAR & 1) != 0
            fl[x] = pwb_u2{fa[x].z, fa[x].w};
#else
            fl[x] = __builtin_amdgcn_raw_buffer_load_b64(rsw, a_lane8, s0 + 2048u + 512u * (unsigned)x, 0);
#endif
#if (PWBK_VAR & 2) != 0
            fa[x] = pwb_u4{a_lane16 + (unsigned)c, a_lane8, s0, a_lane16 ^ s0};
            fl[x] = pwb_u2{fa[x].z, fa[x].w};
#endif
        }
    };
    struct Tup { pwb_u4 hm, mh, lh; };
    auto make = [&](int cl, const XRegs& r) {
        pwb_f4 g01 = {1.0f, 0.0f, 1.0f, 0.0f}, g23 = g01;
        if constexpr (PRO != 0) {
            const float* gp = gnL + 2 * (8 * cl + 4 * half);
            g01 = *reinterpret_cast<const pwb_f4*>(gp);
            g23 = *reinterpret_cast<const pwb_f4*>(gp + 4);
        }
        float v[4];
#pragma unroll
        for (int k = 0; k < 4; ++k) {
            float e = r.x[k];
            if constexpr (PRO != 0) {
                const float sc = k == 0 ? g01.x : (k == 1 ? g01.z : (k == 2 ? g23.x : g23.z));
                const float sh = k == 0 ? g01.y : (k == 1 ? g01.w : (k == 2 ? g23.y : g23.w));
                e = e * sc + sh;
// ... 203 lines not shown
        }
    };
    auto chunk = [&](int c, const pwb_u4 (&fa)[CB], const pwb_u2 (&fl)[CB]) {
#pragma unroll
        for (int nb = 0; nb < NB; ++nb) {
            const pwb_u4 hm = *reinterpret_cast<const pwb_u4*>(S_hm + ((size_t)(c * NB + nb) * 64 + lane) * 4);
            const pwb_u2 lo = *reinterpret_cast<const pwb_u2*>(S_lo + ((size_t)(c * NB + nb) * 64 + lane) * 2);
            const pwb_u4 mh = {hm.z, hm.w, hm.x, hm.y}, lh = {lo.x, lo.y, hm.x, hm.y};
#pragma unroll
            for (int x = 0; x < CB; ++x) {
                const pwb_u4 a_hl = {fa[x].x, fa[x].y, fl[x].x, fl[x].y};
                acc[x][nb] = __builtin_amdgcn_mfma_f32_32x32x16_bf16(__builtin_bit_cast(pwb_bf16x8, fa[x]), __builtin_bit_cast(pwb_bf16x8, hm), acc[x][nb], 0, 0, 0);
                acc[x][nb] = __builtin_amdgcn_mfma_f32_32x32x16_bf16(__builtin_bit_cast(pwb_bf16x8, fa[x]), __builtin_bit_cast(pwb_bf16x8, mh), acc[x][nb], 0, 0, 0);
                acc[x][nb] = __builtin_amdgcn_mfma_f32_32x32x16_bf16(__builtin_bit_cast(pwb_bf16x8, a_hl), __builtin_bit_cast(pwb_bf16x8, lh), acc[x][nb], 0, 0, 0);
            }
        }
    };
    load_f(0, ua, ul);
    if (n > 1) load_f(1, ub, um);
    {
        int c = 0;
        for (; c + 1 < n; c += 2) {
            chunk(c, ua, ul);
            if (c + 2 < n) load_f(c + 2, ua, ul);
            chunk(c + 1, ub, um);
            if (c + 3 < n) load_f(c + 3, ub, um);
        }
        if (c < n) chunk(c, ua, ul);
    }

    const __amdgpu_buffer_rsrc_t rso = __builtin_amdgcn_make_buffer_rsrc(p.out + (size_t)b * p.Cout * HW, 0, -1, 0x00020000);
    const __amdgpu_buffer_rsrc_t rsr = __builtin_amdgcn_make_buffer_rsrc(
        const_cast<float*>(p.residual ? p.residual + (size_t)b * p.Cout * HW : p.out), 0, -1, 0x00020000);
    const unsigned o_voff = 4u * (unsigned)((4 * half) * HW + px0 + NB * l31);
    const int slots = HW / 32;
#pragma unroll
    for (int x = 0; x < CB; ++x) {
        float add[16];
        pwb_f2 res[16];
#pragma unroll
        for (int r = 0; r < 16; ++r) {
            const int cs = co0 + 32 * x + 8 * (r >> 2) + (r & 3);
            const int col = cs + 4 * half;
            add[r] = 0.0f;
            if (p.bias) add[r] += p.bias[col];
            if (p.chan_bias) add[r] += p.chan_bias[(size_t)b * p.chan_bias_stride + col];
            res[r] = pwb_f2{0.0f, 0.0f};
            if (p.residual) res[r] = __builtin_bit_cast(pwb_f2, __builtin_amdgcn_raw_buffer_load_b64(rsr, o_voff, 4u * (unsigned)(cs * HW), 0));
        }
#pragma unroll
        for (int r = 0; r < 16; ++r) {
            const int cs = co0 + 32 * x + 8 * (r >> 2) + (r & 3);
            float vv[2];
#pragma unroll
            for (int nb = 0; nb < NB; ++nb) {
                vv[nb] = acc[x][nb][r] + add[r] + (nb ? res[r].y : res[r].x);
                if (p.relu) vv[nb] = fmaxf(vv[nb], 0.0f);
            }
            __builtin_amdgcn_raw_buffer_store_b64(pwb_u2{__float_as_uint(vv[0]), __float_as_uint(vv[1])}, rso, o_voff, 4u * (unsigned)(cs * HW), 0);
            if (p.stats) {
                const int co = cs + 4 * half;
                const float s1 = pwb_row16_sum(vv[0] + vv[1]);
                const float mean = s1 * (1.0f / 32.0f);
                const float d0 = vv[0] - mean, d1 = vv[1] - mean;
                float q0, q1;
                asm volatile("v_mul_f32 %0, %2, %2\n\tv_mul_f32 %1, %3, %3" : "=&v"(q0), "=&v"(q1) : "v"(d0), "v"(d1));
                const float q = pwb_row16_sum(q0 + q1);
                if ((l31 & 15) == 0)
                    reinterpret_cast<float4*>(p.stats)[((size_t)b * p.Cout + co) * slots + 2 * px_t + (l31 >> 4)] = make_float4(32.0f, s1, q, 0.0f);
            }
        }
    }
}

static bool pwbk_on() { static const bool on = [] { const char* e = std::getenv("SISIC_POINTWISE_KSPLIT"); return !e || std::atoi(e) != 0; }(); return on; }
template <int PRO>
static int launch_pwbk(sisic_ctx* ctx, PwbParams& p, int Cin, hipStream_t s) {
    p.n_co_items = p.Cout / 64;
    p.n_px = p.HW / 32;
    const int64_t nitems = (int64_t)p.B * p.n_px * p.n_co_items;
    SISIC_REQUIRE(nitems > 0 && nitems < (int64_t(1) << 31), "conv2d(pointwise bf16x3, K-split): grid too large");
    p.nitems = (int)nitems;
    p.nwg = p.nitems;
    const size_t lds = sizeof(float) * (size_t)(PWB_WAVES * 32 * 64 + (PRO ? 2 * Cin : 0));
    static std::atomic<uint64_t> opt{0};
    auto kern = conv_pwbk_kernel<PRO>;
    SISIC_TRY(ensure_dynamic_lds(ctx, reinterpret_cast<const void*>(kern), (int)lds, opt));
    hipLaunchKernelGGL(kern, dim3(p.nwg), dim3(64 * PWB_WAVES), lds, s, p);
    SISIC_HIP(hipGetLastError());
    return SISIC_OK;
}

static size_t pwbs_lds_bytes(int Cin) { return (size_t)(Cin / 8) * 2 * 64 * 24 + 8 * (size_t)Cin; }
static bool pwbs_applicable(const sisic_conv_args& a) {
    const int items = a.Cout / 64;
    return items >= 6 && items <= PWBS_MAX_WAVES && pwbs_lds_bytes(a.c0 + a.c1) <= 150 * 1024;
}
template <int PRO>
static int launch_pwbs(sisic_ctx* ctx, PwbParams& p, int Cin, hipStream_t s) {
    p.n_co_items = p.Cout / 64;
    p.n_px = p.HW / 64;
    const int64_t nwg = (int64_t)p.B * p.n_px;
    SISIC_REQUIRE(nwg > 0 && nwg < (int64_t(1) << 31), "conv2d(pointwise bf16x3, staged): grid too large");
    p.nwg = (int)nwg;
    p.nitems = p.nwg * p.n_co_items;
    const size_t lds = pwbs_lds_bytes(Cin);
    static std::atomic<uint64_t> opt{0};
    auto kern = conv_pwbs_kernel<PRO>;
    SISIC_TRY(ensure_dynamic_lds(ctx, reinterpret_cast<const void*>(kern), (int)lds, opt));
    hipLaunchKernelGGL(kern, dim3(p.nwg), dim3(64 * p.n_co_items), lds, s, p);
    SISIC_HIP(hipGetLastError());
    return SISIC_OK;
}

bool conv_pointwise_bf3_applicable(const sisic_conv_args& a) {
    if (a.ksize != 1 || a.stride != 1 || a.upsample) return false;
    const int HW = a.Hin * a.Win, Cin = a.c0 + a.c1;
    if (HW % 64 != 0 || Cin % 8 != 0 || (a.c1 != 0 && a.c0 % 8 != 0) || a.Cout % 64 != 0) return false;
    if (((reinterpret_cast<uintptr_t>(a.in0) | reinterpret_cast<uintptr_t>(a.in1) | reinterpret_cast<uintptr_t>(a.out) |
          reinterpret_cast<uintptr_t>(a.residual)) & 7) != 0) return false;
    if (4.0 * std::max(std::max(a.c0, a.c1), a.Cout) * HW >= 4294967296.0 || 6.0 * conv_cin_pad(Cin, 1) * conv_cout_pad(a.Cout) >= 4294967296.0) return false;
    if (a.gn_scale && Cin > 1024) return false;
    return true;
}

template <int PRO, int NB>
static int launch_pwb(sisic_ctx* ctx, PwbParams& p, int Cin, hipStream_t s) {
    p.n_co_items = p.Cout / 64;
    p.n_px = p.HW / (32 * NB);
    const int64_t nitems = (int64_t)p.B * p.n_px * p.n_co_items;
    SISIC_REQUIRE(nitems > 0 && nitems < (int64_t(1) << 31), "conv2d(pointwise bf16x3): grid too large");
    p.nitems = (int)nitems;
    p.nwg = (int)((nitems + PWB_WAVES - 1) / PWB_WAVES);
    const size_t lds = PRO ? sizeof(float) * (size_t)(PWB_WAVES * 2 * Cin) : 0;
    static std::atomic<uint64_t> opt{0};
    auto kern = conv_pwb_kernel<PRO, NB>;
    SISIC_TRY(ensure_dynamic_lds(ctx, reinterpret_cast<const void*>(kern), (int)lds, opt));
    hipLaunchKernelGGL(kern, dim3(p.nwg), dim3(64 * PWB_WAVES), lds, s, p);
    SISIC_HIP(hipGetLastError());
    return SISIC_OK;
}

int launch_conv_pointwise_bf3(sisic_ctx* ctx, const sisic_conv_args& a, hipStream_t s) {
    SISIC_REQUIRE(conv_pointwise_bf3_applicable(a), "conv2d(pointwise bf16x3): shape not supported by tile_cfg 28");
    PwbParams p{};
    const int Cin = a.c0 + a.c1;
    p.in0 = a.in0; p.in1 = a.in1; p.c0 = a.c0; p.c1 = a.c1; p.B = a.B; p.HW = a.Hin * a.Win;
    p.wb = a.w_packed + 2 * (size_t)conv_cin_pad(Cin, 1) * conv_cout_pad(a.Cout);
    p.n_co64 = conv_cout_pad(a.Cout) / 64;
    p.bias = a.bias; p.Cout = a.Cout;
    p.gn_scale = a.gn_scale; p.gn_shift = a.gn_shift;
    p.chan_bias = a.chan_bias; p.chan_bias_stride = a.chan_bias_stride; p.residual = a.residual; p.relu = a.relu;
    p.out = a.out; p.stats = a.stats_out;
    p.nchunks = Cin / 8;
    const int pro = a.gn_scale == nullptr ? 0 : (a.gn_silu ? 2 : 1);
    {
        const bool ks_ok = p.nchunks % (4 * PWB_WAVES) == 0;
        if (a.tile_cfg == 35) SISIC_REQUIRE(ks_ok, "conv2d(pointwise bf16x3, K-split): tile_cfg 35 needs a multiple of 128 input channels");
        if (a.tile_cfg == 35 || (a.tile_cfg == 0 && ks_ok && p.HW <= 256 && a.Cout <= 256 && pwbk_on())) {
            if (pro == 2) return launch_pwbk<2>(ctx, p, Cin, s);
            if (pro == 1) return launch_pwbk<1>(ctx, p, Cin, s);
            return launch_pwbk<0>(ctx, p, Cin, s);
        }
    }
    if (a.tile_cfg == 34) SISIC_REQUIRE(pwbs_applicable(a), "conv2d(pointwise bf16x3, staged): tile_cfg 34 needs 384 .. 768 output channels and at most %d input channels", (150 * 1024) / 392);
    if (a.tile_cfg == 34 || (a.tile_cfg == 0 && pwbs_applicable(a) && (int64_t)a.B * (p.HW / 64) >= 128)) {
        if (pro == 2) return launch_pwbs<2>(ctx, p, Cin, s);
        if (pro == 1) return launch_pwbs<1>(ctx, p, Cin, s);
        return launch_pwbs<0>(ctx, p, Cin, s);
    }
    const bool wide = a.tile_cfg == 29 ? false : (a.tile_cfg == 30 ? true : (int64_t)a.B * (p.HW / 64) * (a.Cout / 64) >= 2048);
    if (wide) {
        if (pro == 2) return launch_pwb<2, 2>(ctx, p, Cin, s);
        if (pro == 1) return launch_pwb<1, 2>(ctx, p, Cin, s);
        return launch_pwb<0, 2>(ctx, p, Cin, s);
    }
    if (pro == 2) return launch_pwb<2, 1>(ctx, p, Cin, s);
    if (pro == 1) return launch_pwb<1, 1>(ctx, p, Cin, s);
    return launch_pwb<0, 1>(ctx, p, Cin, s);
}

}
```

synt_isic_amd/csrc/groupnorm.hip:

```cpp
#include "common.h"
#include "gn_merge.h"

namespace sisic {

constexpr int GN_THREADS = 256;

__device__ __forceinline__ float wave_sum(float v) {
#pragma unroll
    for (int o = 32; o > 0; o >>= 1) v += __shfl_xor(v, o, 64);
    return v;
}

__device__ __forceinline__ float block_sum(float v, float* red) {
    v = wave_sum(v);
    const int lane = threadIdx.x & 63, wave = threadIdx.x >> 6;
    __syncthreads();
    if (lane == 0) red[wave] = v;
    __syncthreads();
    float t = 0.0f;
#pragma unroll
    for (int w = 0; w < GN_THREADS / 64; ++w) t += red[w];
    return t;
}

__global__ void __launch_bounds__(GN_THREADS)
gn_stats_kernel(const float* __restrict__ in0, int c0, const float* __restrict__ in1, int c1, int HW, int groups,
                float eps, const float* __restrict__ gamma, const float* __restrict__ beta,
                float* __restrict__ scale, float* __restrict__ shift, int aligned16, float* __restrict__ mean_rstd) {
    __shared__ float red[GN_THREADS / 64];
    const int C = c0 + c1;
    const int cpg = C / groups;
    const int b = blockIdx.x / groups, g = blockIdx.x % groups;
    const int tid = threadIdx.x;
    const bool vec = aligned16 && (HW & 3) == 0;

    auto plane = [&](int c) -> const float* {
        return (c < c0) ? in0 + ((size_t)b * c0 + c) * HW : in1 + ((size_t)b * c1 + (c - c0)) * HW;
    };

    const float K = plane(g * cpg)[0];
    float s1 = 0.0f, s2 = 0.0f;
    for (int j = 0; j < cpg; ++j) {
        const float* src = plane(g * cpg + j);
        if (vec) {
            const float4* s4 = reinterpret_cast<const float4*>(src);
            const int n4 = HW / 4;
            int i = tid;
            for (; i + 3 * GN_THREADS < n4; i += 4 * GN_THREADS) {
                const float4 v0 = s4[i], v1 = s4[i + GN_THREADS], v2 = s4[i + 2 * GN_THREADS], v3 = s4[i + 3 * GN_THREADS];
                const float4 vv[4] = {v0, v1, v2, v3};
#pragma unroll
                for (int u = 0; u < 4; ++u) {
                    const float a = vv[u].x - K, bq = vv[u].y - K, c = vv[u].z - K, d = vv[u].w - K;
                    s1 += (a + bq) + (c + d);
                    s2 += (a * a + bq * bq) + (c * c + d * d);
                }
            }
            for (; i < n4; i += GN_THREADS) {
                const float4 v = s4[i];
                const float a = v.x - K, bq = v.y - K, c = v.z - K, d = v.w - K;
                s1 += (a + bq) + (c + d);
                s2 += (a * a + bq * bq) + (c * c + d * d);
            }
        } else {
            for (int i = tid; i < HW; i += GN_THREADS) {
                const float a = src[i] - K;
                s1 += a;
                s2 += a * a;
            }
        }
    }
    const float n = (float)cpg * (float)HW;
    const float m1 = block_sum(s1, red) / n;
    const float m2 = block_sum(s2, red) / n;
    const float mean = K + m1;
    const float var = fmaxf(m2 - m1 * m1, 0.0f);
    const float rstd = 1.0f / sqrtf(var + eps);
    if (mean_rstd && tid == 0) {
        mean_rstd[2 * (size_t)blockIdx.x] = mean;
        mean_rstd[2 * (size_t)blockIdx.x + 1] = rstd;
    }
    if (tid < cpg) {
        const int c = g * cpg + tid;
        const float sc = gamma[c] * rstd;
        scale[(size_t)b * C + c] = sc;
        shift[(size_t)b * C + c] = beta[c] - mean * sc;
    }
}

int launch_gn_stats(sisic_ctx* ctx, const float* in0, int c0, const float* in1, int c1, int B, int HW, int groups,
                    float eps, const float* gamma, const float* beta, float* scale, float* shift, hipStream_t s,
                    float* mean_rstd) {
    SISIC_REQUIRE(in0 && gamma && beta && scale && shift, "groupnorm_stats: null tensor");
    SISIC_REQUIRE((c1 == 0) == (in1 == nullptr), "groupnorm_stats: in1/c1 mismatch");
    const int C = c0 + c1;
    SISIC_REQUIRE(B > 0 && HW > 0 && groups > 0 && C % groups == 0, "groupnorm_stats: C=%d not divisible by groups=%d", C, groups);
    SISIC_REQUIRE(C / groups <= GN_THREADS, "groupnorm_stats: %d channels per group unsupported", C / groups);
    ProfileScope prof(ctx, s, PK_GN, 4.0 * B * C * HW + 8.0 * B * C, 0.0);
    const int aligned16 = ((reinterpret_cast<uintptr_t>(in0) | reinterpret_cast<uintptr_t>(in1)) & 15) == 0;
    hipLaunchKernelGGL(gn_stats_kernel, dim3(B * groups), dim3(GN_THREADS), 0, s, in0, c0, in1, c1, HW, groups, eps,
                       gamma, beta, scale, shift, aligned16, mean_rstd);
    SISIC_HIP(hipGetLastError());
    return SISIC_OK;
}

__device__ __forceinline__ double dpp_f64(double v, const int ctrl_sel) {
    const long long b = __double_as_longlong(v);
    int lo = (int)(b & 0xffffffffll), hi = (int)(b >> 32);
    switch (ctrl_sel) {
        case 0: lo = __builtin_amdgcn_update_dpp(0, lo, 0xB1, 0xf, 0xf, true); hi = __builtin_amdgcn_update_dpp(0, hi, 0xB1, 0xf, 0xf, true); break;
        case 1: lo = __builtin_amdgcn_update_dpp(0, lo, 0x4E, 0xf, 0xf, true); hi = __builtin_amdgcn_update_dpp(0, hi, 0x4E, 0xf, 0xf, true); break;
        case 2: lo = __builtin_amdgcn_update_dpp(0, lo, 0x141, 0xf, 0xf, true); hi = __builtin_amdgcn_update_dpp(0, hi, 0x141, 0xf, 0xf, true); break;
        default: lo = __builtin_amdgcn_update_dpp(0, lo, 0x140, 0xf, 0xf, true); hi = __builtin_amdgcn_update_dpp(0, hi, 0x140, 0xf, 0xf, true); break;
    }
    return __longlong_as_double(((long long)hi << 32) | (unsigned int)lo);
}
__device__ __forceinline__ double wave64_sum_f64(double v) {
    v += dpp_f64(v, 0);
    v += dpp_f64(v, 1);
    v += dpp_f64(v, 2);
    v += dpp_f64(v, 3);
    const long long b = __double_as_longlong(v);
    const int lo = (int)(b & 0xffffffffll), hi = (int)(b >> 32);
    double r[4];
#pragma unroll
    for (int i = 0; i < 4; ++i)
        r[i] = __longlong_as_double(((long long)__builtin_amdgcn_readlane(hi, 16 * i) << 32) |
                                    (unsigned int)__builtin_amdgcn_readlane(lo, 16 * i));
    return (r[0] + r[1]) + (r[2] + r[3]);
}

constexpr int GNF_WAVES = 4;
__global__ void __launch_bounds__(64 * GNF_WAVES) gn_finalize_kernel(const float4* __restrict__ st0, int c0, int slots0,
                                                         const float4* __restrict__ st1, int c1, int slots1,
                                                         int groups, int n_jobs, float eps, const float* __restrict__ gamma,
                                                         const float* __restrict__ beta, float* __restrict__ scale,
                                                         float* __restrict__ shift, float* __restrict__ mean_rstd) {
    const int C = c0 + c1, gs = C / groups;
    const int job = blockIdx.x * GNF_WAVES + (threadIdx.x >> 6);
    if (job >= n_jobs) return;
    const int b = job / groups, g = job % groups;
    const int lane = threadIdx.x & 63;
    const int ca = g * gs, cb = ca + gs;
    const int a0 = min(ca, c0), b0 = min(cb, c0);
    const int a1 = max(ca, c0) - c0, b1 = max(cb, c0) - c0;
    const float4* run0 = st0 + ((size_t)b * c0 + a0) * slots0;
    const int len0 = (b0 - a0) * slots0;
    const float4* run1 = st1 ? st1 + ((size_t)b * c1 + a1) * slots1 : nullptr;
    const int len1 = st1 ? (b1 - a1) * slots1 : 0;
    const float my_gamma = lane < gs ? gamma[ca + lane] : 0.0f, my_beta = lane < gs ? beta[ca + lane] : 0.0f;
    constexpr int KEEP = 4;
    float4 k0[KEEP], k1[KEEP];
    double n = 0.0, s1 = 0.0, m2 = 0.0;
#pragma unroll
    for (int j = 0; j < KEEP; ++j) {
        const int i = lane + 64 * j;
        k0[j] = i < len0 ? run0[i] : make_float4(0.f, 0.f, 0.f, 0.f);
        k1[j] = i < len1 ? run1[i] : make_float4(0.f, 0.f, 0.f, 0.f);
    }
#pragma unroll
    for (int j = 0; j < KEEP; ++j) {
        n += (double)k0[j].x + (double)k1[j].x;
        s1 += (double)k0[j].y + (double)k1[j].y;
        m2 += (double)k0[j].z + (double)k1[j].z;
    }
    for (int i = lane + 64 * KEEP; i < len0; i += 64) { const float4 v = run0[i]; n += v.x; s1 += v.y; m2 += v.z; }
    for (int i = lane + 64 * KEEP; i < len1; i += 64) { const float4 v = run1[i]; n += v.x; s1 += v.y; m2 += v.z; }
    n = wave64_sum_f64(n);
    s1 = wave64_sum_f64(s1);
    m2 = wave64_sum_f64(m2);
    const double mean = s1 / n;
    double between = 0.0;
    auto dev = [&](const float4 v) { between += gn_between_term(v.x, v.y, mean); };
#pragma unroll
    for (int j = 0; j < KEEP; ++j) { dev(k0[j]); dev(k1[j]); }
    for (int i = lane + 64 * KEEP; i < len0; i += 64) dev(run0[i]);
    for (int i = lane + 64 * KEEP; i < len1; i += 64) dev(run1[i]);
    between = wave64_sum_f64(between);
    float meanf, rstd;
    gn_mean_rstd(n, s1, m2, between, eps, meanf, rstd, mean);
    if (mean_rstd && lane == 0) {
        mean_rstd[2 * (size_t)job] = meanf;
        mean_rstd[2 * (size_t)job + 1] = rstd;
    }
    if (lane < gs) {
        float sc, sh;
        gn_affine(my_gamma, my_beta, meanf, rstd, sc, sh);
        scale[(size_t)b * C + ca + lane] = sc;
        shift[(size_t)b * C + ca + lane] = sh;
    }
    for (int cc = lane + 64; cc < gs; cc += 64) {
        const int c = ca + cc;
        float sc, sh;
        gn_affine(gamma[c], beta[c], meanf, rstd, sc, sh);
        scale[(size_t)b * C + c] = sc;
        shift[(size_t)b * C + c] = sh;
    }
}

int launch_gn_finalize(sisic_ctx* ctx, const float* st0, int c0, int slots0, const float* st1, int c1, int slots1, int B,
                       int HW, int groups, float eps, const float* gamma, const float* beta, float* scale, float* shift,
                       hipStream_t s, float* mean_rstd) {
    SISIC_REQUIRE(st0 && gamma && beta && scale && shift, "groupnorm_finalize: null tensor");
    SISIC_REQUIRE((c1 == 0) == (st1 == nullptr), "groupnorm_finalize: stats1/c1 mismatch");
    const int C = c0 + c1;
    SISIC_REQUIRE(B > 0 && HW > 0 && groups > 0 && c0 > 0 && C % groups == 0 && slots0 > 0 && (c1 == 0 || slots1 > 0),
                  "groupnorm_finalize: C=%d groups=%d slots=%d/%d", C, groups, slots0, slots1);
    (void)HW;
    ProfileScope prof(ctx, s, PK_GN, 16.0 * B * (c0 * (double)slots0 + c1 * (double)slots1) + 8.0 * B * C, 0.0);
    hipLaunchKernelGGL(gn_finalize_kernel, dim3(cdiv(B * groups, GNF_WAVES)), dim3(64 * GNF_WAVES), 0, s,
                       reinterpret_cast<const float4*>(st0), c0, slots0, reinterpret_cast<const float4*>(st1), c1, slots1, groups,
                       B * groups, eps, gamma, beta, scale, shift, mean_rstd);
    SISIC_HIP(hipGetLastError());
    return SISIC_OK;
}

}
```

synt_isic_amd/csrc/unet.cpp:

```cpp
#include <algorithm>
#include <cmath>
#include <cstdlib>
#include <cstring>
#include <map>
#include <memory>

#include "unet_internal.h"

using namespace sisic;

namespace {

void add_conv(sisic_unet* u, ConvW& c, const std::string& name, int cout, int cin, int k) {
    c.cout = cout; c.cin = cin; c.k = k;
    c.w_idx = u->add(name + ".weight", (int64_t)cout * cin * k * k);
    c.b_idx = u->add(name + ".bias", cout);
}
void add_norm(sisic_unet* u, NormW& n, const std::string& name, int c) {
    n.c = c;
    n.w_idx = u->add(name + ".weight", c);
    n.b_idx = u->add(name + ".bias", c);
}
void add_resnet(sisic_unet* u, ResnetW& r, const std::string& name, int cin, int cout) {
    r.cin = cin; r.cout = cout;
    add_norm(u, r.norm1, name + ".norm1", cin);
    add_conv(u, r.conv1, name + ".conv1", cout, cin, 3);
    r.temb_w_idx = u->add(name + ".time_emb_proj.weight", (int64_t)cout * u->hidden);
    r.temb_b_idx = u->add(name + ".time_emb_proj.bias", cout);
    r.temb_off = u->tproj_R;
    u->tproj_R += cout;
    add_norm(u, r.norm2, name + ".norm2", cout);
    add_conv(u, r.conv2, name + ".conv2", cout, cout, 3);
    if (cin != cout) add_conv(u, r.shortcut, name + ".conv_shortcut", cout, cin, 1);
    u->max_c = std::max(u->max_c, std::max(cin, cout));
}
void add_attn(sisic_unet* u, AttnW& a, const std::string& name, int c) {
    a.c = c;
    add_norm(u, a.norm, name + ".group_norm", c);
    a.q_w = u->add(name + ".to_q.weight", (int64_t)c * c); a.q_b = u->add(name + ".to_q.bias", c);
    a.k_w = u->add(name + ".to_k.weight", (int64_t)c * c); a.k_b = u->add(name + ".to_k.bias", c);
    a.v_w = u->add(name + ".to_v.weight", (int64_t)c * c); a.v_b = u->add(name + ".to_v.bias", c);
    add_conv(u, a.out, name + ".to_out.0", c, c, 1);
    u->max_c = std::max(u->max_c, c);
}

int describe(sisic_unet* u) {
    const sisic_unet_config& cfg = u->cfg;
    const int n = cfg.n_blocks;
    const int* boc = cfg.block_out_channels;
    u->hidden = 4 * boc[0];
    add_conv(u, u->conv_in, "conv_in", boc[0], cfg.in_channels, 3);
    u->temb_w1 = u->add("time_embedding.linear_1.weight", (int64_t)u->hidden * boc[0]);
    u->temb_b1 = u->add("time_embedding.linear_1.bias", u->hidden);
    u->temb_w2 = u->add("time_embedding.linear_2.weight", (int64_t)u->hidden * u->hidden);
    u->temb_b2 = u->add("time_embedding.linear_2.bias", u->hidden);

    u->down_res.resize(n); u->down_attn.resize(n); u->downsamplers.resize(n);
    int out_ch = boc[0];
    for (int i = 0; i < n; ++i) {
        const int in_ch = out_ch;
        out_ch = boc[i];
        u->down_res[i].resize(cfg.layers_per_block);
        if (cfg.down_attn[i]) u->down_attn[i].resize(cfg.layers_per_block);
        for (int j = 0; j < cfg.layers_per_block; ++j) {
            const std::string base = "down_blocks." + std::to_string(i);
            add_resnet(u, u->down_res[i][j], base + ".resnets." + std::to_string(j), j == 0 ? in_ch : out_ch, out_ch);
            if (cfg.down_attn[i]) add_attn(u, u->down_attn[i][j], base + ".attentions." + std::to_string(j), out_ch);
        }
        if (i != n - 1)
            add_conv(u, u->downsamplers[i], "down_blocks." + std::to_string(i) + ".downsamplers.0.conv", out_ch, out_ch, 3);
    }
    const int mid = boc[n - 1];
    add_resnet(u, u->mid_res[0], "mid_block.resnets.0", mid, mid);
    add_attn(u, u->mid_attn, "mid_block.attentions.0", mid);
    add_resnet(u, u->mid_res[1], "mid_block.resnets.1", mid, mid);

    u->up_res.resize(n); u->up_attn.resize(n); u->upsamplers.resize(n);
    out_ch = boc[n - 1];
    for (int i = 0; i < n; ++i) {
        const int prev_out = out_ch;
        out_ch = boc[n - 1 - i];
        const int in_ch = boc[n - 1 - std::min(i + 1, n - 1)];
        const int layers = cfg.layers_per_block + 1;
        u->up_res[i].resize(layers);
        if (cfg.up_attn[i]) u->up_attn[i].resize(layers);
        for (int j = 0; j < layers; ++j) {
            const int skip_ch = (j == layers - 1) ? in_ch : out_ch;
            const int res_in = (j == 0) ? prev_out : out_ch;
            const std::string base = "up_blocks." + std::to_string(i);
// ... 167 lines not shown
    *out = static_cast<float*>(p);
    return SISIC_OK;
}

void pool_put(sisic_unet* u, float* p) {
    for (auto& b : u->pool)
        if (b.p == p) { b.free_ = true; return; }
}

int grow(float** p, size_t* have, size_t want) {
    if (*have >= want) return SISIC_OK;
    if (*p) SISIC_HIP(hipFree(*p));
    *p = nullptr; *have = 0;
    void* q = nullptr;
    SISIC_HIP(hipMalloc(&q, want * sizeof(float)));
    *p = static_cast<float*>(q);
    *have = want;
    return SISIC_OK;
}

int ensure_rows(sisic_unet* u, size_t t_rows, size_t gn_rows) {
    SISIC_TRY(grow(&u->t_vals, &u->t_vals_cap, t_rows));
    SISIC_TRY(grow(&u->temb_act, &u->temb_act_cap, t_rows * u->hidden));
    SISIC_TRY(grow(&u->tproj, &u->tproj_cap, t_rows * u->tproj_R));
    SISIC_TRY(grow(&u->gn_scale, &u->gn_scale_cap, gn_rows * u->max_c));
    SISIC_TRY(grow(&u->gn_shift, &u->gn_shift_cap, gn_rows * u->max_c));
    SISIC_TRY(grow(&u->gn_scale2, &u->gn_scale2_cap, gn_rows * u->max_c));
    SISIC_TRY(grow(&u->gn_shift2, &u->gn_shift2_cap, gn_rows * u->max_c));
    return SISIC_OK;
}

int stage_upload(sisic_unet* u, const float* src, size_t n, float* dst, hipStream_t s) {
    if (u->stage_cap < n) {
        SISIC_HIP(hipDeviceSynchronize());
        if (u->stage_host) SISIC_HIP(hipHostFree(u->stage_host));
        u->stage_host = nullptr;
        const size_t cap = std::max<size_t>(n, 1024);
        void* p = nullptr;
        SISIC_HIP(hipHostMalloc(&p, cap * sisic_unet::STAGE_SLOTS * sizeof(float), hipHostMallocDefault));
        u->stage_host = static_cast<float*>(p);
        u->stage_cap = cap;
        for (int i = 0; i < sisic_unet::STAGE_SLOTS; ++i) u->stage_used[i] = false;
    }
    const int slot = (int)(u->stage_next++ % sisic_unet::STAGE_SLOTS);
    if (!u->stage_ev[slot]) SISIC_HIP(hipEventCreateWithFlags(&u->stage_ev[slot], hipEventDisableTiming));
    if (u->stage_used[slot]) SISIC_HIP(hipEventSynchronize(u->stage_ev[slot]));
    float* h = u->stage_host + (size_t)slot * u->stage_cap;
    std::memcpy(h, src, n * sizeof(float));
    SISIC_HIP(hipMemcpyAsync(dst, h, n * sizeof(float), hipMemcpyHostToDevice, s));
    SISIC_HIP(hipEventRecord(u->stage_ev[slot], s));
    u->stage_used[slot] = true;
    return SISIC_OK;
}

struct Fwd {
    sisic_unet* u;
    hipStream_t s;
    int B;
    const float* tproj;
    int tproj_stride;
    std::vector<std::unique_ptr<Buf>> bufs;
    TrainState* tr = nullptr;
    float* gsc = nullptr;
    float* gsh = nullptr;
    float* gmr = nullptr;
    const NormW* gnorm = nullptr;

    Buf* make(int C, int H, int W, int* rc) {
        auto b = std::make_unique<Buf>();
        b->C = C; b->H = H; b->W = W; b->refs = 1;
        *rc = pool_get(u, (size_t)B * C * H * W, &b->p);
        bufs.push_back(std::move(b));
        return bufs.back().get();
    }
    void release(Buf* b) {
        if (tr) return;
        if (b && --b->refs == 0 && b->p) {
            pool_put(u, b->p);
            b->p = nullptr;
            if (b->stats) { pool_put(u, b->stats); b->stats = nullptr; }
        }
    }

    int gn(const Buf* x, const Buf* skip, const NormW& n) {
        gsc = u->gn_scale; gsh = u->gn_shift; gmr = nullptr; gnorm = &n;
        if (!tr && !skip && x->fin_norm == static_cast<const void*>(&n)) {
            gsc = x->fin_scale; gsh = x->fin_shift;
            return SISIC_OK;
        }
        if (tr) {
            const int C = x->C + (skip ? skip->C : 0);
            SISIC_TRY(pool_get(u, (size_t)B * C, &gsc));
            SISIC_TRY(pool_get(u, (size_t)B * C, &gsh));
            SISIC_TRY(pool_get(u, (size_t)B * u->cfg.norm_groups * 2, &gmr));
            tr->grads_of_bufs.push_back(gsc); tr->grads_of_bufs.push_back(gsh); tr->grads_of_bufs.push_back(gmr);
        }
        if (x->stats && (!skip || skip->stats))
            return launch_gn_finalize(u->ctx, x->stats, x->C, x->slots, skip ? skip->stats : nullptr, skip ? skip->C : 0,
                                      skip ? skip->slots : 0, B, x->H * x->W, u->cfg.norm_groups, u->cfg.norm_eps,
                                      n.gamma, n.beta, gsc, gsh, s, gmr);
        return launch_gn_stats(u->ctx, x->p, x->C, skip ? skip->p : nullptr, skip ? skip->C : 0, B, x->H * x->W,
                               u->cfg.norm_groups, u->cfg.norm_eps, n.gamma, n.beta, gsc, gsh, s, gmr);
    }

    int conv(const ConvW& c, const float* in0, int c0, const float* in1, int c1, int H, int W, int stride, int ups,
             bool gn_prologue, bool silu, const float* chan_bias, const float* residual, float* out,
             Buf* normed_later = nullptr, Buf* xb = nullptr, Buf* skipb = nullptr, Buf* resb = nullptr, Buf* outb = nullptr,
             const AttnW* qkv_of = nullptr, const NormW* next_norm = nullptr) {
        sisic_conv_args a{};
        a.in0 = in0; a.c0 = c0; a.in1 = in1; a.c1 = c1;
        a.B = B; a.Hin = H; a.Win = W; a.upsample = ups; a.ksize = c.k; a.stride = stride;
        a.w_packed = c.packed; a.bias = c.bias; a.Cout = c.cout;
        a.w_winograd = stride == 1 ? (u->use_winograd ? c.wino : nullptr) : (stride == 2 ? c.s2 : nullptr);
        if (gn_prologue) { a.gn_scale = gsc; a.gn_shift = gsh; a.gn_silu = silu ? 1 : 0; }
        a.chan_bias = chan_bias; a.chan_bias_stride = tproj_stride;
        a.residual = residual; a.out = out;
        if (u->latency_mode) {
            if (c.k == 3 && stride == 1 && !ups && a.w_winograd && c.cout > 4 && H >= 12 && W >= 12) a.tile_cfg = 79;
            else if (c.k == 1 && stride == 1) a.tile_cfg = 22;
            else if (c.k == 3 && stride == 2) a.tile_cfg = 18;
        }
        if (normed_later && u->fuse_gn) {
            const int slots = conv_stats_slots(a);
            if (slots > 0) {
                SISIC_TRY(pool_get(u, (size_t)B * c.cout * slots * 4, &normed_later->stats));
                normed_later->slots = slots;
                a.stats_out = normed_later->stats;
            }
        }
        if (normed_later && next_norm && u->fuse_gn && !tr) {
            a.fin_gamma = next_norm->gamma; a.fin_beta = next_norm->beta; a.fin_groups = u->cfg.norm_groups; a.fin_eps = u->cfg.norm_eps;
            const bool first_pair_busy = gn_prologue && gsc == u->gn_scale;
            a.fin_scale = first_pair_busy ? u->gn_scale2 : u->gn_scale;
            a.fin_shift = first_pair_busy ? u->gn_shift2 : u->gn_shift;
            if (conv_finalizes(a)) { normed_later->fin_norm = next_norm; normed_later->fin_scale = a.fin_scale; normed_later->fin_shift = a.fin_shift; }
            else { a.fin_gamma = nullptr; a.fin_beta = nullptr; a.fin_scale = nullptr; a.fin_shift = nullptr; }
        }
        if (tr) {
            TapeOp op;
            op.kind = TapeOp::CONV;
            op.w = c; op.qkv_of = qkv_of;
            op.in0 = xb; op.in1 = skipb; op.in0_ptr = in0; op.in1_ptr = in1;
            op.c0 = c0; op.c1 = c1; op.H = H; op.W = W; op.stride = stride; op.ups = ups;
            if (gn_prologue) { op.norm = gnorm; op.gn_scale = gsc; op.gn_shift = gsh; op.gn_mr = gmr; op.silu = silu; }
            op.temb_off = chan_bias ? (int)(chan_bias - tproj) : -1;
            op.residual = resb; op.out = outb; op.out_ptr = out;
            tr->tape.push_back(op);
        }
        return launch_conv2d(u->ctx, a, s);
    }

    int resnet(const ResnetW& r, const Buf* x, const Buf* skip, Buf** out, const NormW* next_norm = nullptr) {
        int rc = SISIC_OK;
        const int H = x->H, W = x->W;
        const int c1 = skip ? skip->C : 0;
        SISIC_REQUIRE(x->C + c1 == r.cin, "unet: resnet expects %d input channels, got %d", r.cin, x->C + c1);
        SISIC_TRY(gn(x, skip, r.norm1));
        Buf* h = make(r.cout, H, W, &rc); SISIC_TRY(rc);
        SISIC_TRY(conv(r.conv1, x->p, x->C, skip ? skip->p : nullptr, c1, H, W, 1, 0, true, true,
                       tproj + r.temb_off, nullptr, h->p, h, const_cast<Buf*>(x), const_cast<Buf*>(skip), nullptr, h, nullptr, &r.norm2));
        const float* residual = x->p;
        Buf* resb = const_cast<Buf*>(x);
        Buf* sc = nullptr;
        if (r.shortcut.k) {
            sc = make(r.cout, H, W, &rc); SISIC_TRY(rc);
            SISIC_TRY(conv(r.shortcut, x->p, x->C, skip ? skip->p : nullptr, c1, H, W, 1, 0, false, false, nullptr,
                           nullptr, sc->p, nullptr, const_cast<Buf*>(x), const_cast<Buf*>(skip), nullptr, sc));
            residual = sc->p;
            resb = sc;
        } else {
            SISIC_REQUIRE(c1 == 0 && x->C == r.cout, "unet: identity shortcut with mismatched channels");
        }
        SISIC_TRY(gn(h, nullptr, r.norm2));
        Buf* o = make(r.cout, H, W, &rc); SISIC_TRY(rc);
        SISIC_TRY(conv(r.conv2, h->p, r.cout, nullptr, 0, H, W, 1, 0, true, true, nullptr, residual, o->p, o, h, nullptr,
                       resb, o, nullptr, next_norm));
        release(h);
        release(sc);
        *out = o;
        return SISIC_OK;
    }

    int attention(const AttnW& a, const Buf* x, Buf** out) {
        int rc = SISIC_OK;
        const int H = x->H, W = x->W, N = H * W, C = a.c;
        SISIC_REQUIRE(x->C == C, "unet: attention channel mismatch");
        SISIC_TRY(gn(x, nullptr, a.norm));
        Buf* qkv = make(3 * C, H, W, &rc); SISIC_TRY(rc);
        ConvW cq; cq.cout = 3 * C; cq.cin = C; cq.k = 1; cq.packed = a.qkv_packed; cq.bias = a.qkv_bias;
        SISIC_TRY(conv(cq, x->p, C, nullptr, 0, H, W, 1, 0, true, false, nullptr, nullptr, qkv->p, nullptr,
                       const_cast<Buf*>(x), nullptr, nullptr, qkv, &a));
        Buf* o = make(C, H, W, &rc); SISIC_TRY(rc);
        SISIC_TRY(launch_attention(u->ctx, qkv->p, o->p, B, C, N, u->cfg.head_dim, s));
        if (tr) {
            TapeOp op;
            op.kind = TapeOp::ATTN;
            op.qkv = qkv; op.o = o; op.C = C; op.N = N;
            tr->tape.push_back(op);
        }
        release(qkv);
        Buf* y = make(C, H, W, &rc); SISIC_TRY(rc);
        SISIC_TRY(conv(a.out, o->p, C, nullptr, 0, H, W, 1, 0, false, false, nullptr, x->p, y->p, y, o, nullptr,
                       const_cast<Buf*>(x), y));
        release(o);
        *out = y;
        return SISIC_OK;
    }

    int run(const float* sample, float* out, int H, int W) {
        const sisic_unet_config& cfg = u->cfg;
        const int n = cfg.n_blocks;
        int rc = SISIC_OK;
        std::vector<Buf*> skips;

        Buf* x = make(u->conv_in.cout, H, W, &rc); SISIC_TRY(rc);
        SISIC_TRY(conv(u->conv_in, sample, cfg.in_channels, nullptr, 0, H, W, 1, 0, false, false, nullptr, nullptr, x->p, x,
                       nullptr, nullptr, nullptr, x));
        x->refs++;
        skips.push_back(x);

        for (int i = 0; i < n; ++i) {
            for (int j = 0; j < cfg.layers_per_block; ++j) {
                Buf* y = nullptr;
                const NormW* next = cfg.down_attn[i] ? &u->down_attn[i][j].norm
                                    : (j + 1 < cfg.layers_per_block ? &u->down_res[i][j + 1].norm1 : (i == n - 1 ? &u->mid_res[0].norm1 : nullptr));
                SISIC_TRY(resnet(u->down_res[i][j], x, nullptr, &y, next));
                release(x);
                x = y;
                if (cfg.down_attn[i]) {
                    SISIC_TRY(attention(u->down_attn[i][j], x, &y));
                    release(x);
                    x = y;
                }
                x->refs++;
                skips.push_back(x);
            }
            if (i != n - 1) {
                const int Ho = (x->H + 2 - 3) / 2 + 1, Wo = (x->W + 2 - 3) / 2 + 1;
                Buf* y = make(u->downsamplers[i].cout, Ho, Wo, &rc); SISIC_TRY(rc);
                SISIC_TRY(conv(u->downsamplers[i], x->p, x->C, nullptr, 0, x->H, x->W, 2, 0, false, false, nullptr, nullptr, y->p, y,
                               x, nullptr, nullptr, y));
                release(x);
                x = y;
                x->refs++;
                skips.push_back(x);
            }
        }
// ... 42 lines not shown
    }
};

int check_shape(sisic_unet* u, int B, int H, int W) {
    SISIC_REQUIRE(u, "unet: null handle");
    if (!u->loaded) {
        set_error("unet: forward called before sisic_unet_load");
        return SISIC_ESTATE;
    }
    SISIC_HIP(hipSetDevice(u->ctx->device));
    const int div = 1 << (u->cfg.n_blocks - 1);
    SISIC_REQUIRE(B > 0 && H > 0 && W > 0 && H % div == 0 && W % div == 0,
                  "unet: sample %dx%dx%d unsupported (H and W must be positive multiples of %d)", B, H, W, div);
    if (u->ws_B != B || u->ws_H != H || u->ws_W != W) {
        SISIC_HIP(hipDeviceSynchronize());
        pool_release_all(u);
        u->ws_B = B; u->ws_H = H; u->ws_W = W;
    }
    return SISIC_OK;
}

int time_embed(sisic_unet* u, int rows, hipStream_t s) {
    SISIC_TRY(launch_temb_mlp(u->ctx, u->t_vals, rows, u->d_freqs, u->cfg.n_freqs, u->w1t, u->rawp(u->temb_b1), u->w2t,
                              u->rawp(u->temb_b2), u->hidden, u->temb_act, s));
    SISIC_TRY(launch_linear_t(u->ctx, u->temb_act, rows, u->hidden, u->tproj_wt, u->tproj_b, u->tproj_R, u->tproj, s));
    return SISIC_OK;
}

int run_forward(sisic_unet* u, const float* sample, const float* tproj, int tproj_stride, float* out, int B, int H,
                int W, hipStream_t s, TrainState* tr = nullptr) {
    Fwd f{u, s, B, tproj, tproj_stride, {}};
    f.tr = tr;
    f.gsc = u->gn_scale; f.gsh = u->gn_shift;
    const int rc = f.run(sample, out, H, W);
    if (tr && rc == SISIC_OK) {
        for (auto& b : f.bufs) tr->bufs.push_back(std::move(b));
        return rc;
    }
    for (auto& b : f.bufs) {
        if (b->p) pool_put(u, b->p);
        if (b->stats) pool_put(u, b->stats);
    }
    if (tr) tr->tape.clear();
    return rc;
}

}

namespace sisic {
int unet_pool_get(sisic_unet* u, size_t floats, float** out) { return pool_get(u, floats, out); }
void unet_release_tape(sisic_unet* u) { tape_drop(u, true); }
void unet_pool_put(sisic_unet* u, float* p) { pool_put(u, p); }
int unet_grow(float** p, size_t* have, size_t want) { return grow(p, have, want); }
int unet_check_shape(sisic_unet* u, int B, int H, int W) { return check_shape(u, B, H, W); }
int unet_ensure_rows(sisic_unet* u, size_t t_rows, size_t gn_rows) { return ensure_rows(u, t_rows, gn_rows); }
int unet_stage_upload(sisic_unet* u, const float* src, size_t n, float* dst, hipStream_t s) { return stage_upload(u, src, n, dst, s); }
int unet_prepare_all(sisic_unet* u, hipStream_t s) { return prepare_all(u, s); }
int unet_run_forward(sisic_unet* u, const float* sample, const float* tproj, int tproj_stride, float* out, int B, int H,
                     int W, hipStream_t s, TrainState* tape) {
    return run_forward(u, sample, tproj, tproj_stride, out, B, H, W, s, tape);
}
}

extern "C" {

int sisic_unet_create(sisic_ctx* ctx, const sisic_unet_config* cfg, sisic_unet** out) {
    SISIC_REQUIRE(ctx && cfg && out, "unet_create: null argument");
    *out = nullptr;
    SISIC_REQUIRE(cfg->n_blocks >= 1 && cfg->n_blocks <= 8, "unet_create: n_blocks %d", cfg->n_blocks);
    SISIC_REQUIRE(cfg->layers_per_block >= 1, "unet_create: layers_per_block");
    SISIC_REQUIRE(cfg->in_channels > 0 && cfg->out_channels > 0, "unet_create: channels");
    SISIC_REQUIRE(cfg->norm_groups > 0 && cfg->head_dim == 8, "unet_create: head_dim must be 8, groups > 0");
    SISIC_REQUIRE(cfg->freqs && cfg->n_freqs * 2 == cfg->block_out_channels[0], "unet_create: freqs table must hold block_out_channels[0]/2 entries");
    for (int i = 0; i < cfg->n_blocks; ++i)
        SISIC_REQUIRE(cfg->block_out_channels[i] > 0 && cfg->block_out_channels[i] % cfg->norm_groups == 0 &&
                          cfg->block_out_channels[i] % cfg->head_dim == 0,
                      "unet_create: block_out_channels[%d]=%d", i, cfg->block_out_channels[i]);
    auto* u = new sisic_unet();
    u->ctx = ctx;
    u->cfg = *cfg;
    u->freqs.assign(cfg->freqs, cfg->freqs + cfg->n_freqs);
    if (const char* e = std::getenv("SISIC_WINOGRAD")) u->use_winograd = std::atoi(e) != 0;
    if (const char* e = std::getenv("SISIC_FUSED_GN")) u->fuse_gn = std::atoi(e) != 0;
    if (const char* e = std::getenv("SISIC_GRAPH")) u->graph_mode = std::atoi(e) != 0 ? 1 : 0;
    u->cfg.freqs = nullptr;
    const int rc = describe(u);
    if (rc != SISIC_OK) { delete u; return rc; }
    *out = u;
    return SISIC_OK;
}

int sisic_unet_destroy(sisic_unet* u) {
    if (!u) return SISIC_OK;
    (void)sisic_unet_train_end(u);
    (void)hipDeviceSynchronize();
    pool_release_all(u);
    for (float* p : {u->x_work, u->loop_tables, u->tproj_cur, u->seeds_dev})
        if (p) (void)hipFree(p);
    if (u->loop_stream) (void)hipStreamDestroy(u->loop_stream);
    for (auto p : u->owned) (void)hipFree(p);
    for (float* p : {u->raw, u->t_vals, u->temb_act, u->tproj, u->gn_scale, u->gn_shift, u->gn_scale2, u->gn_shift2, u->eps_buf})
        if (p) (void)hipFree(p);
    if (u->stage_host) (void)hipHostFree(u->stage_host);
    for (auto e : u->stage_ev)
        if (e) (void)hipEventDestroy(e);
    delete u;
    return SISIC_OK;
}

int sisic_unet_set_latency_mode(sisic_unet* u, int on) {
    SISIC_REQUIRE(u, "set_latency_mode: null handle");
    u->latency_mode = on != 0;
    return SISIC_OK;
}

int sisic_unet_set_graph_mode(sisic_unet* u, int mode) {
    SISIC_REQUIRE(u && mode >= -1 && mode <= 1, "set_graph_mode: mode must be -1 (follow latency mode), 0 or 1");
    u->graph_mode = mode;
    return SISIC_OK;
}

int64_t sisic_unet_graph_builds(const sisic_unet* u) { return u ? u->loop_builds : 0; }

int64_t sisic_unet_workspace_bytes(const sisic_unet* u) {
    int64_t n = 0;
    if (u) for (const auto& b : u->pool) n += (int64_t)b.bytes;
    return n;
}

int sisic_unet_num_tensors(const sisic_unet* u) { return u ? (int)u->names.size() : 0; }

const char* sisic_unet_tensor_name(const sisic_unet* u, int i) {
    if (!u || i < 0 || i >= (int)u->names.size()) return nullptr;
    return u->names[i].c_str();
}

int sisic_unet_load(sisic_unet* u, int n, const char* const* names, const float* const* host_ptrs,
                    const int64_t* numels) {
    SISIC_REQUIRE(u && names && host_ptrs && numels, "unet_load: null argument");
    SISIC_REQUIRE(n == (int)u->names.size(), "unet_load: state dict has %d tensors, expected %d", n, (int)u->names.size());
    SISIC_HIP(hipSetDevice(u->ctx->device));
    if (!u->raw) {
        void* p = nullptr;
        SISIC_HIP(hipMalloc(&p, u->raw_floats * sizeof(float)));
        u->raw = static_cast<float*>(p);
    }
    SISIC_HIP(hipMemset(u->raw, 0, u->raw_floats * sizeof(float)));
    std::vector<char> seen(u->names.size(), 0);
    for (int i = 0; i < n; ++i) {
        SISIC_REQUIRE(names[i] && host_ptrs[i], "unet_load: entry %d is null", i);
        auto it = u->index.find(names[i]);
        SISIC_REQUIRE(it != u->index.end(), "unet_load: unexpected key '%s'", names[i]);
        const int idx = it->second;
        SISIC_REQUIRE(!seen[idx], "unet_load: duplicate key '%s'", names[i]);
        SISIC_REQUIRE(numels[i] == u->numels[idx], "unet_load: '%s' has %lld elements, expected %lld", names[i],
                      (long long)numels[i], (long long)u->numels[idx]);
        seen[idx] = 1;
        SISIC_HIP(hipMemcpy(u->raw + u->offsets[idx], host_ptrs[i], (size_t)numels[i] * sizeof(float), hipMemcpyHostToDevice));
    }
    SISIC_HIP(hipDeviceSynchronize());
    loop_graph_drop(u);
    for (auto p : u->owned) (void)hipFree(p);
    u->owned.clear();
    reset_derived(u);
    u->loaded = false;
    SISIC_TRY(prepare_all(u, nullptr));
// ... 220 lines not shown
```

synt_isic_amd/csrc/unet_internal.h:

```cpp
#pragma once

#include <map>
#include <memory>
#include <string>
#include <vector>

#include "common.h"

namespace sisic {

struct ConvW {
    int cout = 0, cin = 0, k = 0;
    int w_idx = -1, b_idx = -1;
    float* packed = nullptr;
    float* wino = nullptr;
    bool strided = false;
    float* s2 = nullptr;
    const float* bias = nullptr;
    float* raw_t = nullptr;
    float* packed_t = nullptr;
    float* wino_t = nullptr;
};

struct NormW {
// ... 73 lines not shown
    std::vector<std::unique_ptr<Buf>> bufs;
    std::vector<float*> grads_of_bufs;
    std::map<const Buf*, float*> buf_grad;
    int B = 0, H = 0, W = 0;
    bool has_tape = false;
    float* emb = nullptr;
    float* h1 = nullptr;
    float* t2 = nullptr;
    size_t emb_cap = 0, h1_cap = 0, t2_cap = 0;
    float* dtproj = nullptr;
    size_t dtproj_cap = 0;
    float* garena = nullptr;
    size_t garena_cap = 0, garena_used = 0;
    float* wgrad_part = nullptr;
    size_t wgrad_part_cap = 0;
    float* scratch = nullptr;
    size_t scratch_cap = 0;
    float* small = nullptr;
    size_t small_cap = 0;
    float* loss_dev = nullptr;
    int* flag_dev = nullptr;
    float* mse_part = nullptr;
    void* repack_dev[3] = {nullptr, nullptr, nullptr};
    int repack_jobs[3] = {0, 0, 0}, repack_blocks[3] = {0, 0, 0};
    void* scatter_dev = nullptr;
    int scatter_jobs = 0, scatter_blocks = 0;
    const float* scatter_src = nullptr;
    bool repack_ready = false;
};

}

struct sisic_unet {
    using ConvW = sisic::ConvW; using NormW = sisic::NormW; using ResnetW = sisic::ResnetW; using AttnW = sisic::AttnW;
    using PoolBlock = sisic::PoolBlock;
    sisic_ctx* ctx = nullptr;
    sisic_unet_config cfg{};
    std::vector<float> freqs;

    std::vector<std::string> names;
    std::vector<int64_t> numels;
    std::vector<size_t> offsets;
    std::map<std::string, int> index;
    float* raw = nullptr;
    size_t raw_floats = 0;
    std::vector<float*> owned;
    bool loaded = false;

    ConvW conv_in, conv_out;
    NormW norm_out;
    int temb_w1 = -1, temb_b1 = -1, temb_w2 = -1, temb_b2 = -1;
    float* d_freqs = nullptr;
    float* w1t = nullptr;
    float* w2t = nullptr;
    float* tproj_wt = nullptr;
    float* tproj_b = nullptr;
    int hidden = 0, tproj_R = 0;
    std::vector<std::vector<ResnetW>> down_res, up_res;
    std::vector<std::vector<AttnW>> down_attn, up_attn;
    std::vector<ConvW> downsamplers, upsamplers;
    ResnetW mid_res[2];
    AttnW mid_attn;
    int max_c = 0;

    std::vector<PoolBlock> pool;
    int ws_B = 0, ws_H = 0, ws_W = 0;
    float* t_vals = nullptr;
    float* temb_act = nullptr;
    float* tproj = nullptr;
    float* gn_scale = nullptr;
    float* gn_shift = nullptr;
    float* gn_scale2 = nullptr;
    float* gn_shift2 = nullptr;
    size_t t_vals_cap = 0, temb_act_cap = 0, tproj_cap = 0, gn_scale_cap = 0, gn_shift_cap = 0, gn_scale2_cap = 0, gn_shift2_cap = 0;
    static constexpr int STAGE_SLOTS = 4;
    float* stage_host = nullptr;
    size_t stage_cap = 0;
    uint64_t stage_next = 0;
    hipEvent_t stage_ev[STAGE_SLOTS] = {};
    bool stage_used[STAGE_SLOTS] = {};
    bool latency_mode = false;
    bool use_winograd = true;
    bool fuse_gn = true;
    float* eps_buf = nullptr;
    size_t eps_floats = 0;
    std::unique_ptr<sisic::TrainState> train;

    int graph_mode = -1;
    hipGraph_t loop_graph = nullptr;
    hipGraphExec_t loop_exec = nullptr;
    struct LoopKey {
        int B = 0, H = 0, W = 0; float clip = 0; hipStream_t s = nullptr; bool latency = false; uint64_t gen = 0;
        const void* ptrs[5] = {};
        bool rng = false;
        const void* seeds = nullptr;
    } loop_key;
    bool loop_valid = false;
    int64_t loop_builds = 0;
    hipStream_t loop_stream = nullptr;
    float* x_work = nullptr;
    size_t x_work_cap = 0;
    float* loop_tables = nullptr;
    size_t loop_tables_cap = 0;
    float* tproj_cur = nullptr;
    size_t tproj_cur_cap = 0;
    float* seeds_dev = nullptr;
    size_t seeds_cap = 0;

    int add(const std::string& name, int64_t numel) {
        index[name] = (int)names.size();
        names.push_back(name);
        numels.push_back(numel);
        return (int)names.size() - 1;
    }
    const float* rawp(int idx) const { return raw + offsets[idx]; }
};


namespace sisic {

int unet_pool_get(sisic_unet* u, size_t floats, float** out);
void unet_pool_put(sisic_unet* u, float* p);
void unet_release_tape(sisic_unet* u);
inline size_t train_small_floats(const sisic_unet* u, int B) {
    return (size_t)B * 5 * (size_t)u->max_c + 3 * (size_t)u->max_c + 2 * (size_t)B;
}
int unet_grow(float** p, size_t* have, size_t want);
int unet_check_shape(sisic_unet* u, int B, int H, int W);
int unet_ensure_rows(sisic_unet* u, size_t t_rows, size_t gn_rows);
int unet_stage_upload(sisic_unet* u, const float* src, size_t n, float* dst, hipStream_t s);
int unet_prepare_all(sisic_unet* u, hipStream_t s);
int unet_run_forward(sisic_unet* u, const float* sample, const float* tproj, int tproj_stride, float* out, int B, int H,
                     int W, hipStream_t s, TrainState* tape);

inline std::vector<ResnetW*> unet_resnets(sisic_unet* u) {
    std::vector<ResnetW*> v;
    for (auto& blk : u->down_res) for (auto& r : blk) v.push_back(&r);
    for (auto& r : u->mid_res) v.push_back(&r);
    for (auto& blk : u->up_res) for (auto& r : blk) v.push_back(&r);
    return v;
}
inline std::vector<AttnW*> unet_attns(sisic_unet* u) {
    std::vector<AttnW*> v;
    for (auto& blk : u->down_attn) for (auto& a : blk) v.push_back(&a);
    v.push_back(&u->mid_attn);
    for (auto& blk : u->up_attn) for (auto& a : blk) v.push_back(&a);
    return v;
}
inline std::vector<ConvW*> unet_convs(sisic_unet* u) {
    std::vector<ConvW*> v{&u->conv_in, &u->conv_out};
    for (auto* r : unet_resnets(u)) {
        v.push_back(&r->conv1); v.push_back(&r->conv2);
        if (r->shortcut.k) v.push_back(&r->shortcut);
    }
    for (auto* a : unet_attns(u)) v.push_back(&a->out);
    for (auto& c : u->downsamplers) if (c.k) v.push_back(&c);
    for (auto& c : u->upsamplers) if (c.k) v.push_back(&c);
    return v;
}

}
```

synt_isic_amd/ops.py:

```python
from __future__ import annotations

import ctypes as C
from typing import Optional

import numpy as np
import torch

from . import _lib
from ._lib import ConvArgs, check

_ctx_by_device = {}


def context(device: torch.device) -> C.c_void_p:
    device = torch.device(device)
    if device.type != "cuda":
        raise RuntimeError(f"synt_isic_amd runs on MI355X (torch device 'cuda'); got '{device}'. There is no CPU path.")
    idx = device.index if device.index is not None else torch.cuda.current_device()
    if idx not in _ctx_by_device:
        lib = _lib.load()
        h = C.c_void_p()
        check(lib.sisic_create(idx, C.byref(h)))
        _ctx_by_device[idx] = h
    return _ctx_by_device[idx]
# ... 25 lines not shown
    return out


def pack_winograd_weight(w: torch.Tensor) -> torch.Tensor:
    lib = _lib.load()
    cout, cin, k, k2 = w.shape
    if k != 3 or k2 != 3:
        raise ValueError("Winograd F(2x2,3x3) needs a 3x3 weight")
    out = torch.empty(lib.sisic_conv_winograd_numel(cout, cin), dtype=torch.float32, device=w.device)
    check(lib.sisic_conv_winograd_pack(context(w.device), _ptr(w, "weight"), cout, cin, out.data_ptr(),
                                       _stream(w.device)))
    return out


def pack_conv_s2_weight(w: torch.Tensor) -> torch.Tensor:
    lib = _lib.load()
    cout, cin, k, k2 = w.shape
    if k != 3 or k2 != 3:
        raise ValueError("the stride-2 bf16x3 kernel needs a 3x3 weight")
    out = torch.empty(lib.sisic_conv_s2_numel(cout, cin), dtype=torch.float32, device=w.device)
    check(lib.sisic_conv_s2_pack(context(w.device), _ptr(w, "weight"), cout, cin, out.data_ptr(), _stream(w.device)))
    return out


def conv2d(x: torch.Tensor, w_packed: torch.Tensor, cout: int, ksize: int, *, bias=None, x2=None, stride=1,
           upsample=False, gn_scale=None, gn_shift=None, gn_silu=False, chan_bias=None, residual=None,
           relu=False, tile_cfg=0, w_winograd=None, with_stats=False, out=None, finalize=None):
    lib = _lib.load()
    B, c0, H, W = x.shape
    c1 = 0 if x2 is None else x2.shape[1]
    Hc, Wc = (2 * H, 2 * W) if upsample else (H, W)
    pad = ksize // 2
    Ho = (Hc + 2 * pad - ksize) // stride + 1
    Wo = (Wc + 2 * pad - ksize) // stride + 1
    if out is None:
        out = torch.empty((B, cout, Ho, Wo), dtype=torch.float32, device=x.device)
    elif tuple(out.shape) != (B, cout, Ho, Wo) or out.dtype != torch.float32 or not out.is_contiguous() or out.device != x.device:
        raise ValueError(f"out must be a contiguous fp32 {(B, cout, Ho, Wo)} tensor on {x.device}")
    a = ConvArgs()
    a.in0 = _ptr(x, "x"); a.in1 = _ptr(x2, "x2"); a.c0 = c0; a.c1 = c1
    a.B = B; a.Hin = H; a.Win = W
    a.upsample = int(upsample); a.ksize = ksize; a.stride = stride
    a.w_packed = _ptr(w_packed, "w_packed"); a.bias = _ptr(bias, "bias"); a.Cout = cout
    a.gn_scale = _ptr(gn_scale, "gn_scale"); a.gn_shift = _ptr(gn_shift, "gn_shift"); a.gn_silu = int(gn_silu)
    a.chan_bias = _ptr(chan_bias, "chan_bias"); a.chan_bias_stride = cout if chan_bias is not None and chan_bias.dim() == 2 and chan_bias.shape[0] == B else 0
    a.residual = _ptr(residual, "residual"); a.relu = int(relu)
    a.out = out.data_ptr(); a.tile_cfg = tile_cfg
    a.w_winograd = _ptr(w_winograd, "w_winograd")
    stats = None
    if with_stats:
        slots = lib.sisic_conv_stats_slots(C.byref(a))
        if slots > 0:
            stats = torch.empty((B, cout, slots, 4), dtype=torch.float32, device=x.device)
            a.stats_out = stats.data_ptr()
    fin = None
    if finalize is not None:
        gamma, beta, groups, eps = finalize
        a.fin_gamma = _ptr(gamma, "gamma"); a.fin_beta = _ptr(beta, "beta"); a.fin_groups = int(groups); a.fin_eps = float(eps)
        if lib.sisic_conv_finalizes(C.byref(a)):
            fin = (torch.empty((B, cout), dtype=torch.float32, device=x.device), torch.empty((B, cout), dtype=torch.float32, device=x.device))
            a.fin_scale, a.fin_shift = fin[0].data_ptr(), fin[1].data_ptr()
        else:
            a.fin_gamma = None
    check(lib.sisic_conv2d(context(x.device), C.byref(a), _stream(x.device)))
    res = (out, stats) if with_stats else out
    if finalize is not None:
        res = (res + (fin,)) if with_stats else (res, fin)
    return res


def groupnorm_finalize(stats: torch.Tensor, hw: int, gamma: torch.Tensor, beta: torch.Tensor, groups: int, eps: float,
                       stats2: Optional[torch.Tensor] = None):
    lib = _lib.load()
    B, c0, slots0, _ = stats.shape
    c1, slots1 = (0, 0) if stats2 is None else (stats2.shape[1], stats2.shape[2])
    scale = torch.empty((B, c0 + c1), dtype=torch.float32, device=stats.device)
    shift = torch.empty_like(scale)
    check(lib.sisic_groupnorm_finalize(context(stats.device), _ptr(stats, "stats"), c0, slots0, _ptr(stats2, "stats2"),
                                       c1, slots1, B, hw, groups, float(eps), _ptr(gamma, "gamma"), _ptr(beta, "beta"),
                                       scale.data_ptr(), shift.data_ptr(), _stream(stats.device)))
    return scale, shift


def groupnorm_stats(x: torch.Tensor, gamma: torch.Tensor, beta: torch.Tensor, groups: int, eps: float,
                    x2: Optional[torch.Tensor] = None):
    lib = _lib.load()
    B, c0 = x.shape[0], x.shape[1]
    c1 = 0 if x2 is None else x2.shape[1]
    HW = x[0, 0].numel()
    scale = torch.empty((B, c0 + c1), dtype=torch.float32, device=x.device)
    shift = torch.empty_like(scale)
    check(lib.sisic_groupnorm_stats(context(x.device), _ptr(x, "x"), c0, _ptr(x2, "x2"), c1, B, HW, groups,
                                    float(eps), _ptr(gamma, "gamma"), _ptr(beta, "beta"), scale.data_ptr(),
                                    shift.data_ptr(), _stream(x.device)))
    return scale, shift


def attention(qkv: torch.Tensor, head_dim: int = 8) -> torch.Tensor:
    lib = _lib.load()
    B, C3, N = qkv.shape
    Cc = C3 // 3
    out = torch.empty((B, Cc, N), dtype=torch.float32, device=qkv.device)
    check(lib.sisic_attention(context(qkv.device), _ptr(qkv, "qkv"), out.data_ptr(), B, Cc, N, head_dim,
                              _stream(qkv.device)))
    return out


def ddpm_step(eps: torch.Tensor, x: torch.Tensor, z: Optional[torch.Tensor], coef, clip: float = 1.0,
              out: Optional[torch.Tensor] = None) -> torch.Tensor:
    lib = _lib.load()
    if out is None:
        out = torch.empty_like(x)
    sb, sa, c0, c1, sigma = (float(v) for v in coef)
    check(lib.sisic_ddpm_step(context(x.device), _ptr(eps, "eps"), _ptr(x, "x"), _ptr(z, "z"), _ptr(out, "out"),
                              x.numel(), sb, sa, c0, c1, sigma, float(clip), _stream(x.device)))
    return out


def _seed_array(seeds):
    seeds = [int(s) for s in seeds]
    if not seeds or any(s < 0 or s >> 64 for s in seeds):
        raise ValueError("seeds must be a non-empty sequence of integers in 0 .. 2**64-1")
    return (C.c_uint64 * len(seeds))(*seeds)


def noise_fill(seeds, n_per_image: int, step: int, tag: int = 0, device="cuda") -> torch.Tensor:
    lib = _lib.load()
    device = torch.device(device)
    arr = _seed_array(seeds)
    out = torch.empty((len(arr), int(n_per_image)), dtype=torch.float32, device=device)
    check(lib.sisic_noise_fill(context(device), out.data_ptr(), len(arr), int(n_per_image), arr, int(step), int(tag),
                               _stream(device)))
    return out


def noise_bits(seeds, n_per_image: int, step: int, tag: int = 0, device="cuda") -> torch.Tensor:
    lib = _lib.load()
    device = torch.device(device)
    arr = _seed_array(seeds)
    words = 4 * ((int(n_per_image) + 3) // 4)
    out = torch.empty((len(arr), words), dtype=torch.int32, device=device)
    check(lib.sisic_noise_bits(context(device), out.data_ptr(), len(arr), int(n_per_image), arr, int(step), int(tag),
                               _stream(device)))
    return out


def ddpm_step_rng(eps: torch.Tensor, x: torch.Tensor, seeds, step: int, coef, clip: float = 1.0,
                  out: Optional[torch.Tensor] = None) -> torch.Tensor:
    lib = _lib.load()
    arr = _seed_array(seeds)
    B = len(arr)
    if x.numel() % B:
        raise ValueError(f"{x.numel()} elements are not {B} equal images")
    if out is None:
        out = torch.empty_like(x)
    seeds_dev = torch.frombuffer(bytearray(bytes(arr)), dtype=torch.int64).to(x.device)
    sb, sa, c0, c1, sigma = (float(v) for v in coef)
    check(lib.sisic_ddpm_step_rng(context(x.device), _ptr(eps, "eps"), _ptr(x, "x"), _ptr(out, "out"), B, x.numel() // B,
                                  seeds_dev.data_ptr(), int(step), sb, sa, c0, c1, sigma, float(clip), _stream(x.device)))
    return out


def conv2d_wgrad(x: torch.Tensor, dy: torch.Tensor, ksize: int, *, x2=None, stride=1, upsample=False, gn_scale=None,
                 gn_shift=None, gn_silu=False) -> torch.Tensor:
    lib = _lib.load()
    B, c0, H, W = x.shape
# ... 203 lines not shown
```

Before: 12.55.

## Run GroupNorm finalize as rider workgroups inside the shortcut pointwise conv launch

In resnet blocks that have a 1x1 shortcut conv, the GroupNorm finalize for norm1 is deferred and its jobs run as extra leading workgroups of the shortcut conv kernel, which has no GN prologue. The shortcut conv is moved ahead of conv1 so it can carry this work, which saves a separate kernel launch and its serialization per affected block. If the conv path cannot take the rider, the code falls back to a standalone finalize launch. The risk is extra grid size and some shifting of workgroup scheduling within the conv.

```diff
diff --git a/include/sisic.h b/include/sisic.h
--- a/include/sisic.h
+++ b/include/sisic.h
@@ -83,6 +83,13 @@
                              const float* gamma, const float* beta,
                              float* scale, float* shift, void* stream);
 
+int sisic_conv2d_gn_rider(sisic_ctx*, const sisic_conv_args* args,
+                          const float* stats0, int c0, int slots0,
+                          const float* stats1, int c1, int slots1,
+                          int B, int HW, int groups, float eps,
+                          const float* gamma, const float* beta,
+                          float* scale, float* shift, int* carried, void* stream);
+
 int sisic_attention(sisic_ctx*, const float* qkv, float* out, int B, int C, int N, int head_dim,
                     void* stream);
 
diff --git a/synt_isic_amd/_lib.py b/synt_isic_amd/_lib.py
--- a/synt_isic_amd/_lib.py
+++ b/synt_isic_amd/_lib.py
@@ -77,6 +77,9 @@
     "sisic_groupnorm_finalize": (C.c_int, [C.c_void_p, C.c_void_p, C.c_int, C.c_int, C.c_void_p, C.c_int, C.c_int,
                                            C.c_int, C.c_int, C.c_int, C.c_float, C.c_void_p, C.c_void_p, C.c_void_p,
                                            C.c_void_p, C.c_void_p]),
+    "sisic_conv2d_gn_rider": (C.c_int, [C.c_void_p, C.POINTER(ConvArgs), C.c_void_p, C.c_int, C.c_int, C.c_void_p, C.c_int,
+                                        C.c_int, C.c_int, C.c_int, C.c_int, C.c_float, C.c_void_p, C.c_void_p, C.c_void_p,
+                                        C.c_void_p, C.POINTER(C.c_int), C.c_void_p]),
     "sisic_groupnorm_stats": (C.c_int, [C.c_void_p, C.c_void_p, C.c_int, C.c_void_p, C.c_int, C.c_int, C.c_int,
                                         C.c_int, C.c_float, C.c_void_p, C.c_void_p, C.c_void_p, C.c_void_p,
                                         C.c_void_p]),
diff --git a/synt_isic_amd/csrc/api.cpp b/synt_isic_amd/csrc/api.cpp
--- a/synt_isic_amd/csrc/api.cpp
+++ b/synt_isic_amd/csrc/api.cpp
@@ -1,6 +1,7 @@
 #include <cstring>
 
 #include "common.h"
+#include "gn_finalize.h"
 
 namespace sisic {
 
@@ -152,6 +153,20 @@
                               shift, static_cast<hipStream_t>(stream));
 }
 
+int sisic_conv2d_gn_rider(sisic_ctx* ctx, const sisic_conv_args* args, const float* stats0, int c0, int slots0,
+                          const float* stats1, int c1, int slots1, int B, int HW, int groups, float eps, const float* gamma,
+                          const float* beta, float* scale, float* shift, int* carried, void* stream) {
+    SISIC_REQUIRE(ctx && args && carried, "conv2d_gn_rider: null argument");
+    *carried = 0;
+    SISIC_REQUIRE(HW > 0, "conv2d_gn_rider: HW=%d", HW);
+    GnFinJob q{};
+    SISIC_TRY(make_gn_fin_job(&q, stats0, c0, slots0, stats1, c1, slots1, B, groups, eps, gamma, beta, scale, shift));
+    bool rode = false;
+    SISIC_TRY(launch_conv2d(ctx, *args, static_cast<hipStream_t>(stream), &q, &rode));
+    *carried = rode ? 1 : 0;
+    return SISIC_OK;
+}
+
 int sisic_groupnorm_stats(sisic_ctx* ctx, const float* in0, int c0, const float* in1, int c1, int B, int HW,
                           int groups, float eps, const float* gamma, const float* beta, float* scale, float* shift,
                           void* stream) {
diff --git a/synt_isic_amd/csrc/common.h b/synt_isic_amd/csrc/common.h
--- a/synt_isic_amd/csrc/common.h
+++ b/synt_isic_amd/csrc/common.h
@@ -115,7 +115,8 @@
     return ksize == 1 ? 3 * first + first / 2 : first;
 }
 
-int launch_conv2d(sisic_ctx*, const sisic_conv_args& a, hipStream_t s);
+struct GnFinJob;
+int launch_conv2d(sisic_ctx*, const sisic_conv_args& a, hipStream_t s, const GnFinJob* rider = nullptr, bool* carried = nullptr);
 int launch_conv_smallcout(sisic_ctx*, const sisic_conv_args& a, hipStream_t s);
 int launch_score_head_bwd(sisic_ctx*, const float* logits, const float* fc_w, const float* act, float* g, int B, int C,
                           int HW, int n_classes, int target, hipStream_t s);
@@ -135,7 +136,8 @@
 int conv_pointwise_stats_slots(const sisic_conv_args& a);
 int launch_conv_pointwise(sisic_ctx*, const sisic_conv_args& a, hipStream_t s);
 bool conv_pointwise_bf3_applicable(const sisic_conv_args& a);
-int launch_conv_pointwise_bf3(sisic_ctx*, const sisic_conv_args& a, hipStream_t s);
+int launch_conv_pointwise_bf3(sisic_ctx*, const sisic_conv_args& a, hipStream_t s, const GnFinJob* rider = nullptr,
+                              bool* carried = nullptr);
 bool conv_s2_bf3_applicable(const sisic_conv_args& a);
 int conv_s2_bf3_stats_slots(const sisic_conv_args& a);
 int launch_conv_s2_bf3(sisic_ctx*, const sisic_conv_args& a, hipStream_t s);
@@ -144,6 +146,9 @@
 int launch_gn_finalize(sisic_ctx*, const float* st0, int c0, int slots0, const float* st1, int c1, int slots1, int B,
                        int HW, int groups, float eps, const float* gamma, const float* beta, float* scale, float* shift,
                        hipStream_t s, float* mean_rstd = nullptr);
+int make_gn_fin_job(GnFinJob* q, const float* st0, int c0, int slots0, const float* st1, int c1, int slots1, int B, int groups,
+                    float eps, const float* gamma, const float* beta, float* scale, float* shift, float* mean_rstd = nullptr);
+int launch_gn_finalize_job(sisic_ctx*, const GnFinJob& q, hipStream_t s);
 int launch_conv_winograd(sisic_ctx*, const sisic_conv_args& a, const float* u_packed, int cfg, hipStream_t s);
 int launch_winograd_pack(sisic_ctx*, const float* w, int Cout, int Cin, float* packed, hipStream_t s);
 int64_t winograd_packed_numel(int Cout, int Cin);
diff --git a/synt_isic_amd/csrc/conv_mfma.hip b/synt_isic_amd/csrc/conv_mfma.hip
--- a/synt_isic_amd/csrc/conv_mfma.hip
+++ b/synt_isic_amd/csrc/conv_mfma.hip
@@ -428,7 +428,8 @@
     return SISIC_OK;
 }
 
-static int dispatch_conv2d(sisic_ctx* ctx, const sisic_conv_args& a, hipStream_t s, int* slots_query);
+static int dispatch_conv2d(sisic_ctx* ctx, const sisic_conv_args& a, hipStream_t s, int* slots_query, const GnFinJob* rider = nullptr,
+                           bool* carried = nullptr);
 
 static int winograd_cfg(const sisic_conv_args& a) {
     if (!(a.ksize == 3 && a.stride == 1 && a.w_winograd != nullptr && a.Cout > 4) || a.upsample == 2) return 0;
@@ -487,9 +488,13 @@
     return ((reinterpret_cast<uintptr_t>(a.residual) | reinterpret_cast<uintptr_t>(a.out) | reinterpret_cast<uintptr_t>(a.stats_out)) & 15) == 0;
 }
 
-int launch_conv2d(sisic_ctx* ctx, const sisic_conv_args& a, hipStream_t s) { return dispatch_conv2d(ctx, a, s, nullptr); }
-
-static int dispatch_conv2d(sisic_ctx* ctx, const sisic_conv_args& a, hipStream_t s, int* slots_query) {
+int launch_conv2d(sisic_ctx* ctx, const sisic_conv_args& a, hipStream_t s, const GnFinJob* rider, bool* carried) {
+    return dispatch_conv2d(ctx, a, s, nullptr, rider, carried);
+}
+
+static int dispatch_conv2d(sisic_ctx* ctx, const sisic_conv_args& a, hipStream_t s, int* slots_query, const GnFinJob* rider,
+                           bool* carried) {
+    if (carried) *carried = false;
     SISIC_REQUIRE(a.in0 && a.w_packed && a.out, "conv2d: null tensor");
     SISIC_REQUIRE(a.B > 0 && a.Hin > 0 && a.Win > 0 && a.c0 > 0 && a.c1 >= 0 && a.Cout > 0, "conv2d: bad shape");
     SISIC_REQUIRE((a.c1 == 0) == (a.in1 == nullptr), "conv2d: in1/c1 mismatch");
@@ -557,7 +562,7 @@
         static const bool pwb_on = [] { const char* e = std::getenv("SISIC_POINTWISE_BF16X3"); return !e || std::atoi(e) != 0; }();
         if ((cfg == 0 && pwb_on && conv_pointwise_bf3_applicable(a)) || (cfg >= 28 && cfg <= 30) || cfg == 34 || cfg == 35) {
             if (slots_query) { *slots_query = conv_pointwise_stats_slots(a); return SISIC_OK; }
-            return launch_conv_pointwise_bf3(ctx, a, s);
+            return launch_conv_pointwise_bf3(ctx, a, s, rider, carried);
         }
         if ((cfg == 0 && pw_on && conv_pointwise_applicable(a)) || cfg == 20) {
             if (slots_query) { *slots_query = conv_pointwise_stats_slots(a); return SISIC_OK; }
diff --git a/synt_isic_amd/csrc/conv_pointwise_bf3.hip b/synt_isic_amd/csrc/conv_pointwise_bf3.hip
--- a/synt_isic_amd/csrc/conv_pointwise_bf3.hip
+++ b/synt_isic_amd/csrc/conv_pointwise_bf3.hip
@@ -2,6 +2,7 @@
 #include <type_traits>
 
 #include "common.h"
+#include "gn_finalize.h"
 
 namespace sisic {
 
@@ -29,6 +30,8 @@
     float* out;
     float* stats;
     int n_px, n_co_items, nitems, nwg, nchunks;
+    int n_rider_wg;
+    GnFinJob rider;
 };
 
 constexpr int PWB_WAVES = 4;
@@ -52,9 +55,17 @@
 template <int PRO, int NB>
 __global__ void __launch_bounds__(64 * PWB_WAVES, 4) conv_pwb_kernel(const PwbParams p) {
     extern __shared__ __attribute__((aligned(16))) float smem[];
+    int L = blockIdx.x;
+    if constexpr (PRO == 0) {
+        if (L < p.n_rider_wg) {
+            gn_finalize_job(p.rider, L * GNF_WAVES + (int)(threadIdx.x >> 6), threadIdx.x & 63);
+            return;
+        }
+        L -= p.n_rider_wg;
+    }
     int wg;
     {
-        const int L = blockIdx.x, nwg = p.nwg;
+        const int nwg = p.nwg;
         const int xcd = L & 7, slot = L >> 3, q = nwg >> 3, r = nwg & 7;
         wg = (xcd < r ? xcd * (q + 1) : r * (q + 1) + (xcd - r) * q) + slot;
     }
@@ -309,9 +320,17 @@
 template <int PRO>
 __global__ void __launch_bounds__(64 * PWB_WAVES, 4) conv_pwbk_kernel(const PwbParams p) {
     extern __shared__ __attribute__((aligned(16))) float smem[];
+    int L = blockIdx.x;
+    if constexpr (PRO == 0) {
+        if (L < p.n_rider_wg) {
+            gn_finalize_job(p.rider, L * GNF_WAVES + (int)(threadIdx.x >> 6), threadIdx.x & 63);
+            return;
+        }
+        L -= p.n_rider_wg;
+    }
     int item;
     {
-        const int L = blockIdx.x, nwg = p.nwg;
+        const int nwg = p.nwg;
         const int xcd = L & 7, slot = L >> 3, q = nwg >> 3, r = nwg & 7;
         item = (xcd < r ? xcd * (q + 1) : r * (q + 1) + (xcd - r) * q) + slot;
     }
@@ -681,11 +700,12 @@
     SISIC_REQUIRE(nitems > 0 && nitems < (int64_t(1) << 31), "conv2d(pointwise bf16x3, K-split): grid too large");
     p.nitems = (int)nitems;
     p.nwg = p.nitems;
+    SISIC_REQUIRE((int64_t)p.nwg + p.n_rider_wg < (int64_t(1) << 31), "conv2d(pointwise bf16x3, K-split): grid too large");
     const size_t lds = sizeof(float) * (size_t)(PWB_WAVES * 32 * 64 + (PRO ? 2 * Cin : 0));
     static std::atomic<uint64_t> opt{0};
     auto kern = conv_pwbk_kernel<PRO>;
     SISIC_TRY(ensure_dynamic_lds(ctx, reinterpret_cast<const void*>(kern), (int)lds, opt));
-    hipLaunchKernelGGL(kern, dim3(p.nwg), dim3(64 * PWB_WAVES), lds, s, p);
+    hipLaunchKernelGGL(kern, dim3(p.n_rider_wg + p.nwg), dim3(64 * PWB_WAVES), lds, s, p);
     SISIC_HIP(hipGetLastError());
     return SISIC_OK;
 }
@@ -731,16 +751,18 @@
     SISIC_REQUIRE(nitems > 0 && nitems < (int64_t(1) << 31), "conv2d(pointwise bf16x3): grid too large");
     p.nitems = (int)nitems;
     p.nwg = (int)((nitems + PWB_WAVES - 1) / PWB_WAVES);
+    SISIC_REQUIRE((int64_t)p.nwg + p.n_rider_wg < (int64_t(1) << 31), "conv2d(pointwise bf16x3): grid too large");
     const size_t lds = PRO ? sizeof(float) * (size_t)(PWB_WAVES * 2 * Cin) : 0;
     static std::atomic<uint64_t> opt{0};
     auto kern = conv_pwb_kernel<PRO, NB>;
     SISIC_TRY(ensure_dynamic_lds(ctx, reinterpret_cast<const void*>(kern), (int)lds, opt));
-    hipLaunchKernelGGL(kern, dim3(p.nwg), dim3(64 * PWB_WAVES), lds, s, p);
+    hipLaunchKernelGGL(kern, dim3(p.n_rider_wg + p.nwg), dim3(64 * PWB_WAVES), lds, s, p);
     SISIC_HIP(hipGetLastError());
     return SISIC_OK;
 }
 
-int launch_conv_pointwise_bf3(sisic_ctx* ctx, const sisic_conv_args& a, hipStream_t s) {
+int launch_conv_pointwise_bf3(sisic_ctx* ctx, const sisic_conv_args& a, hipStream_t s, const GnFinJob* rider, bool* carried) {
+    if (carried) *carried = false;
     SISIC_REQUIRE(conv_pointwise_bf3_applicable(a), "conv2d(pointwise bf16x3): shape not supported by tile_cfg 28");
     PwbParams p{};
     const int Cin = a.c0 + a.c1;
@@ -753,13 +775,22 @@
     p.out = a.out; p.stats = a.stats_out;
     p.nchunks = Cin / 8;
     const int pro = a.gn_scale == nullptr ? 0 : (a.gn_silu ? 2 : 1);
+    static_assert(PWB_WAVES == GNF_WAVES, "a rider workgroup runs one finalisation job per wave");
+    auto with_rider = [&]() {
+        if (rider && carried && pro == 0) { p.rider = *rider; p.n_rider_wg = cdiv(rider->n_jobs, GNF_WAVES); }
+    };
+    auto done = [&](int rc) {
+        if (rc == SISIC_OK && p.n_rider_wg > 0) *carried = true;
+        return rc;
+    };
     {
         const bool ks_ok = p.nchunks % (4 * PWB_WAVES) == 0;
         if (a.tile_cfg == 35) SISIC_REQUIRE(ks_ok, "conv2d(pointwise bf16x3, K-split): tile_cfg 35 needs a multiple of 128 input channels");
         if (a.tile_cfg == 35 || (a.tile_cfg == 0 && ks_ok && p.HW <= 256 && a.Cout <= 256 && pwbk_on())) {
             if (pro == 2) return launch_pwbk<2>(ctx, p, Cin, s);
             if (pro == 1) return launch_pwbk<1>(ctx, p, Cin, s);
-            return launch_pwbk<0>(ctx, p, Cin, s);
+            with_rider();
+            return done(launch_pwbk<0>(ctx, p, Cin, s));
         }
     }
     if (a.tile_cfg == 34) SISIC_REQUIRE(pwbs_applicable(a), "conv2d(pointwise bf16x3, staged): tile_cfg 34 needs 384 .. 768 output channels and at most %d input channels", (150 * 1024) / 392);
@@ -772,11 +803,13 @@
     if (wide) {
         if (pro == 2) return launch_pwb<2, 2>(ctx, p, Cin, s);
         if (pro == 1) return launch_pwb<1, 2>(ctx, p, Cin, s);
-        return launch_pwb<0, 2>(ctx, p, Cin, s);
+        with_rider();
+        return done(launch_pwb<0, 2>(ctx, p, Cin, s));
     }
     if (pro == 2) return launch_pwb<2, 1>(ctx, p, Cin, s);
     if (pro == 1) return launch_pwb<1, 1>(ctx, p, Cin, s);
-    return launch_pwb<0, 1>(ctx, p, Cin, s);
-}
-
-}
+    with_rider();
+    return done(launch_pwb<0, 1>(ctx, p, Cin, s));
+}
+
+}
diff --git a/synt_isic_amd/csrc/gn_finalize.h b/synt_isic_amd/csrc/gn_finalize.h
--- /dev/null
+++ b/synt_isic_amd/csrc/gn_finalize.h
@@ -0,0 +1,120 @@
+#pragma once
+
+#include <hip/hip_runtime.h>
+
+#include "gn_merge.h"
+
+namespace sisic {
+
+constexpr int GNF_WAVES = 4;
+
+struct GnFinJob {
+    const float4* st0;
+    const float4* st1;
+    int c0, slots0, c1, slots1;
+    int groups, n_jobs;
+    float eps;
+    const float* gamma;
+    const float* beta;
+    float* scale;
+    float* shift;
+    float* mean_rstd;
+};
+
+__device__ __forceinline__ double dpp_f64(double v, const int ctrl_sel) {
+    const long long b = __double_as_longlong(v);
+    int lo = (int)(b & 0xffffffffll), hi = (int)(b >> 32);
+    switch (ctrl_sel) {
+        case 0: lo = __builtin_amdgcn_update_dpp(0, lo, 0xB1, 0xf, 0xf, true); hi = __builtin_amdgcn_update_dpp(0, hi, 0xB1, 0xf, 0xf, true); break;
+        case 1: lo = __builtin_amdgcn_update_dpp(0, lo, 0x4E, 0xf, 0xf, true); hi = __builtin_amdgcn_update_dpp(0, hi, 0x4E, 0xf, 0xf, true); break;
+        case 2: lo = __builtin_amdgcn_update_dpp(0, lo, 0x141, 0xf, 0xf, true); hi = __builtin_amdgcn_update_dpp(0, hi, 0x141, 0xf, 0xf, true); break;
+        default: lo = __builtin_amdgcn_update_dpp(0, lo, 0x140, 0xf, 0xf, true); hi = __builtin_amdgcn_update_dpp(0, hi, 0x140, 0xf, 0xf, true); break;
+    }
+    return __longlong_as_double(((long long)hi << 32) | (unsigned int)lo);
+}
+__device__ __forceinline__ double wave64_sum_f64(double v) {
+    v += dpp_f64(v, 0);
+    v += dpp_f64(v, 1);
+    v += dpp_f64(v, 2);
+    v += dpp_f64(v, 3);
+    const long long b = __double_as_longlong(v);
+    const int lo = (int)(b & 0xffffffffll), hi = (int)(b >> 32);
+    double r[4];
+#pragma unroll
+    for (int i = 0; i < 4; ++i)
+        r[i] = __longlong_as_double(((long long)__builtin_amdgcn_readlane(hi, 16 * i) << 32) |
+                                    (unsigned int)__builtin_amdgcn_readlane(lo, 16 * i));
+    return (r[0] + r[1]) + (r[2] + r[3]);
+}
+
+__device__ __forceinline__ void gn_finalize_job(const GnFinJob& q, const int job, const int lane) {
+    const int c0 = q.c0, c1 = q.c1, slots0 = q.slots0, slots1 = q.slots1, groups = q.groups;
+    const float4* __restrict__ st0 = q.st0;
+    const float4* __restrict__ st1 = q.st1;
+    const float* __restrict__ gamma = q.gamma;
+    const float* __restrict__ beta = q.beta;
+    float* __restrict__ scale = q.scale;
+    float* __restrict__ shift = q.shift;
+    float* __restrict__ mean_rstd = q.mean_rstd;
+    const float eps = q.eps;
+    const int C = c0 + c1, gs = C / groups;
+    if (job >= q.n_jobs) return;
+    const int b = job / groups, g = job % groups;
+    const int ca = g * gs, cb = ca + gs;
+    const int a0 = min(ca, c0), b0 = min(cb, c0);
+    const int a1 = max(ca, c0) - c0, b1 = max(cb, c0) - c0;
+    const float4* run0 = st0 + ((size_t)b * c0 + a0) * slots0;
+    const int len0 = (b0 - a0) * slots0;
+    const float4* run1 = st1 ? st1 + ((size_t)b * c1 + a1) * slots1 : nullptr;
+    const int len1 = st1 ? (b1 - a1) * slots1 : 0;
+    const float my_gamma = lane < gs ? gamma[ca + lane] : 0.0f, my_beta = lane < gs ? beta[ca + lane] : 0.0f;
+    constexpr int KEEP = 4;
+    float4 k0[KEEP], k1[KEEP];
+    double n = 0.0, s1 = 0.0, m2 = 0.0;
+#pragma unroll
+    for (int j = 0; j < KEEP; ++j) {
+        const int i = lane + 64 * j;
+        k0[j] = i < len0 ? run0[i] : make_float4(0.f, 0.f, 0.f, 0.f);
+        k1[j] = i < len1 ? run1[i] : make_float4(0.f, 0.f, 0.f, 0.f);
+    }
+#pragma unroll
+    for (int j = 0; j < KEEP; ++j) {
+        n += (double)k0[j].x + (double)k1[j].x;
+        s1 += (double)k0[j].y + (double)k1[j].y;
+        m2 += (double)k0[j].z + (double)k1[j].z;
+    }
+    for (int i = lane + 64 * KEEP; i < len0; i += 64) { const float4 v = run0[i]; n += v.x; s1 += v.y; m2 += v.z; }
+    for (int i = lane + 64 * KEEP; i < len1; i += 64) { const float4 v = run1[i]; n += v.x; s1 += v.y; m2 += v.z; }
+    n = wave64_sum_f64(n);
+    s1 = wave64_sum_f64(s1);
+    m2 = wave64_sum_f64(m2);
+    const double mean = s1 / n;
+    double between = 0.0;
+    auto dev = [&](const float4 v) { between += gn_between_term(v.x, v.y, mean); };
+#pragma unroll
+    for (int j = 0; j < KEEP; ++j) { dev(k0[j]); dev(k1[j]); }
+    for (int i = lane + 64 * KEEP; i < len0; i += 64) dev(run0[i]);
+    for (int i = lane + 64 * KEEP; i < len1; i += 64) dev(run1[i]);
+    between = wave64_sum_f64(between);
+    float meanf, rstd;
+    gn_mean_rstd(n, s1, m2, between, eps, meanf, rstd, mean);
+    if (mean_rstd && lane == 0) {
+        mean_rstd[2 * (size_t)job] = meanf;
+        mean_rstd[2 * (size_t)job + 1] = rstd;
+    }
+    if (lane < gs) {
+        float sc, sh;
+        gn_affine(my_gamma, my_beta, meanf, rstd, sc, sh);
+        scale[(size_t)b * C + ca + lane] = sc;
+        shift[(size_t)b * C + ca + lane] = sh;
+    }
+    for (int cc = lane + 64; cc < gs; cc += 64) {
+        const int c = ca + cc;
+        float sc, sh;
+        gn_affine(gamma[c], beta[c], meanf, rstd, sc, sh);
+        scale[(size_t)b * C + c] = sc;
+        shift[(size_t)b * C + c] = sh;
+    }
+}
+
+}
diff --git a/synt_isic_amd/csrc/groupnorm.hip b/synt_isic_amd/csrc/groupnorm.hip
--- a/synt_isic_amd/csrc/groupnorm.hip
+++ b/synt_isic_amd/csrc/groupnorm.hip
@@ -1,4 +1,5 @@
 #include "common.h"
+#include "gn_finalize.h"
 #include "gn_merge.h"
 
 namespace sisic {
@@ -104,115 +105,40 @@
     return SISIC_OK;
 }
 
-__device__ __forceinline__ double dpp_f64(double v, const int ctrl_sel) {
-    const long long b = __double_as_longlong(v);
-    int lo = (int)(b & 0xffffffffll), hi = (int)(b >> 32);
-    switch (ctrl_sel) {
-        case 0: lo = __builtin_amdgcn_update_dpp(0, lo, 0xB1, 0xf, 0xf, true); hi = __builtin_amdgcn_update_dpp(0, hi, 0xB1, 0xf, 0xf, true); break;
-        case 1: lo = __builtin_amdgcn_update_dpp(0, lo, 0x4E, 0xf, 0xf, true); hi = __builtin_amdgcn_update_dpp(0, hi, 0x4E, 0xf, 0xf, true); break;
-        case 2: lo = __builtin_amdgcn_update_dpp(0, lo, 0x141, 0xf, 0xf, true); hi = __builtin_amdgcn_update_dpp(0, hi, 0x141, 0xf, 0xf, true); break;
-        default: lo = __builtin_amdgcn_update_dpp(0, lo, 0x140, 0xf, 0xf, true); hi = __builtin_amdgcn_update_dpp(0, hi, 0x140, 0xf, 0xf, true); break;
-    }
-    return __longlong_as_double(((long long)hi << 32) | (unsigned int)lo);
-}
-__device__ __forceinline__ double wave64_sum_f64(double v) {
-    v += dpp_f64(v, 0);
-    v += dpp_f64(v, 1);
-    v += dpp_f64(v, 2);
-    v += dpp_f64(v, 3);
-    const long long b = __double_as_longlong(v);
-    const int lo = (int)(b & 0xffffffffll), hi = (int)(b >> 32);
-    double r[4];
-#pragma unroll
-    for (int i = 0; i < 4; ++i)
-        r[i] = __longlong_as_double(((long long)__builtin_amdgcn_readlane(hi, 16 * i) << 32) |
-                                    (unsigned int)__builtin_amdgcn_readlane(lo, 16 * i));
-    return (r[0] + r[1]) + (r[2] + r[3]);
+__global__ void __launch_bounds__(64 * GNF_WAVES) gn_finalize_kernel(const GnFinJob q) {
+    gn_finalize_job(q, blockIdx.x * GNF_WAVES + (threadIdx.x >> 6), threadIdx.x & 63);
 }
 
-constexpr int GNF_WAVES = 4;
-__global__ void __launch_bounds__(64 * GNF_WAVES) gn_finalize_kernel(const float4* __restrict__ st0, int c0, int slots0,
-                                                         const float4* __restrict__ st1, int c1, int slots1,
-                                                         int groups, int n_jobs, float eps, const float* __restrict__ gamma,
-                                                         const float* __restrict__ beta, float* __restrict__ scale,
-                                                         float* __restrict__ shift, float* __restrict__ mean_rstd) {
-    const int C = c0 + c1, gs = C / groups;
-    const int job = blockIdx.x * GNF_WAVES + (threadIdx.x >> 6);
-    if (job >= n_jobs) return;
-    const int b = job / groups, g = job % groups;
-    const int lane = threadIdx.x & 63;
-    const int ca = g * gs, cb = ca + gs;
-    const int a0 = min(ca, c0), b0 = min(cb, c0);
-    const int a1 = max(ca, c0) - c0, b1 = max(cb, c0) - c0;
-    const float4* run0 = st0 + ((size_t)b * c0 + a0) * slots0;
-    const int len0 = (b0 - a0) * slots0;
-    const float4* run1 = st1 ? st1 + ((size_t)b * c1 + a1) * slots1 : nullptr;
-    const int len1 = st1 ? (b1 - a1) * slots1 : 0;
-    const float my_gamma = lane < gs ? gamma[ca + lane] : 0.0f, my_beta = lane < gs ? beta[ca + lane] : 0.0f;
-    constexpr int KEEP = 4;
-    float4 k0[KEEP], k1[KEEP];
-    double n = 0.0, s1 = 0.0, m2 = 0.0;
-#pragma unroll
-    for (int j = 0; j < KEEP; ++j) {
-        const int i = lane + 64 * j;
-        k0[j] = i < len0 ? run0[i] : make_float4(0.f, 0.f, 0.f, 0.f);
-        k1[j] = i < len1 ? run1[i] : make_float4(0.f, 0.f, 0.f, 0.f);
-    }
-#pragma unroll
-    for (int j = 0; j < KEEP; ++j) {
-        n += (double)k0[j].x + (double)k1[j].x;
-        s1 += (double)k0[j].y + (double)k1[j].y;
-        m2 += (double)k0[j].z + (double)k1[j].z;
-    }
-    for (int i = lane + 64 * KEEP; i < len0; i += 64) { const float4 v = run0[i]; n += v.x; s1 += v.y; m2 += v.z; }
-    for (int i = lane + 64 * KEEP; i < len1; i += 64) { const float4 v = run1[i]; n += v.x; s1 += v.y; m2 += v.z; }
-    n = wave64_sum_f64(n);
-    s1 = wave64_sum_f64(s1);
-    m2 = wave64_sum_f64(m2);
-    const double mean = s1 / n;
-    double between = 0.0;
-    auto dev = [&](const float4 v) { between += gn_between_term(v.x, v.y, mean); };
-#pragma unroll
-    for (int j = 0; j < KEEP; ++j) { dev(k0[j]); dev(k1[j]); }
-    for (int i = lane + 64 * KEEP; i < len0; i += 64) dev(run0[i]);
-    for (int i = lane + 64 * KEEP; i < len1; i += 64) dev(run1[i]);
-    between = wave64_sum_f64(between);
-    float meanf, rstd;
-    gn_mean_rstd(n, s1, m2, between, eps, meanf, rstd, mean);
-    if (mean_rstd && lane == 0) {
-        mean_rstd[2 * (size_t)job] = meanf;
-        mean_rstd[2 * (size_t)job + 1] = rstd;
-    }
-    if (lane < gs) {
-        float sc, sh;
-        gn_affine(my_gamma, my_beta, meanf, rstd, sc, sh);
-        scale[(size_t)b * C + ca + lane] = sc;
-        shift[(size_t)b * C + ca + lane] = sh;
-    }
-    for (int cc = lane + 64; cc < gs; cc += 64) {
-        const int c = ca + cc;
-        float sc, sh;
-        gn_affine(gamma[c], beta[c], meanf, rstd, sc, sh);
-        scale[(size_t)b * C + c] = sc;
-        shift[(size_t)b * C + c] = sh;
-    }
+int make_gn_fin_job(GnFinJob* q, const float* st0, int c0, int slots0, const float* st1, int c1, int slots1, int B, int groups,
+                    float eps, const float* gamma, const float* beta, float* scale, float* shift, float* mean_rstd) {
+    SISIC_REQUIRE(st0 && gamma && beta && scale && shift, "groupnorm_finalize: null tensor");
+    SISIC_REQUIRE((c1 == 0) == (st1 == nullptr), "groupnorm_finalize: stats1/c1 mismatch");
+    const int C = c0 + c1;
+    SISIC_REQUIRE(B > 0 && groups > 0 && c0 > 0 && C % groups == 0 && slots0 > 0 && (c1 == 0 || slots1 > 0),
+                  "groupnorm_finalize: C=%d groups=%d slots=%d/%d", C, groups, slots0, slots1);
+    SISIC_REQUIRE((int64_t)B * groups < (int64_t(1) << 31), "groupnorm_finalize: B=%d groups=%d: too many jobs", B, groups);
+    q->st0 = reinterpret_cast<const float4*>(st0); q->st1 = reinterpret_cast<const float4*>(st1);
+    q->c0 = c0; q->slots0 = slots0; q->c1 = c1; q->slots1 = slots1;
+    q->groups = groups; q->n_jobs = B * groups; q->eps = eps;
+    q->gamma = gamma; q->beta = beta; q->scale = scale; q->shift = shift; q->mean_rstd = mean_rstd;
+    return SISIC_OK;
+}
+
+int launch_gn_finalize_job(sisic_ctx* ctx, const GnFinJob& q, hipStream_t s) {
+    const int B = q.n_jobs / q.groups, C = q.c0 + q.c1;
+    ProfileScope prof(ctx, s, PK_GN, 16.0 * B * (q.c0 * (double)q.slots0 + q.c1 * (double)q.slots1) + 8.0 * B * C, 0.0);
+    hipLaunchKernelGGL(gn_finalize_kernel, dim3(cdiv(q.n_jobs, GNF_WAVES)), dim3(64 * GNF_WAVES), 0, s, q);
+    SISIC_HIP(hipGetLastError());
+    return SISIC_OK;
 }
 
 int launch_gn_finalize(sisic_ctx* ctx, const float* st0, int c0, int slots0, const float* st1, int c1, int slots1, int B,
                        int HW, int groups, float eps, const float* gamma, const float* beta, float* scale, float* shift,
                        hipStream_t s, float* mean_rstd) {
-    SISIC_REQUIRE(st0 && gamma && beta && scale && shift, "groupnorm_finalize: null tensor");
-    SISIC_REQUIRE((c1 == 0) == (st1 == nullptr), "groupnorm_finalize: stats1/c1 mismatch");
-    const int C = c0 + c1;
-    SISIC_REQUIRE(B > 0 && HW > 0 && groups > 0 && c0 > 0 && C % groups == 0 && slots0 > 0 && (c1 == 0 || slots1 > 0),
-                  "groupnorm_finalize: C=%d groups=%d slots=%d/%d", C, groups, slots0, slots1);
-    (void)HW;
-    ProfileScope prof(ctx, s, PK_GN, 16.0 * B * (c0 * (double)slots0 + c1 * (double)slots1) + 8.0 * B * C, 0.0);
-    hipLaunchKernelGGL(gn_finalize_kernel, dim3(cdiv(B * groups, GNF_WAVES)), dim3(64 * GNF_WAVES), 0, s,
-                       reinterpret_cast<const float4*>(st0), c0, slots0, reinterpret_cast<const float4*>(st1), c1, slots1, groups,
-                       B * groups, eps, gamma, beta, scale, shift, mean_rstd);
-    SISIC_HIP(hipGetLastError());
-    return SISIC_OK;
+    SISIC_REQUIRE(HW > 0, "groupnorm_finalize: HW=%d", HW);
+    GnFinJob q{};
+    SISIC_TRY(make_gn_fin_job(&q, st0, c0, slots0, st1, c1, slots1, B, groups, eps, gamma, beta, scale, shift, mean_rstd));
+    return launch_gn_finalize_job(ctx, q, s);
 }
 
 }
diff --git a/synt_isic_amd/csrc/unet.cpp b/synt_isic_amd/csrc/unet.cpp
--- a/synt_isic_amd/csrc/unet.cpp
+++ b/synt_isic_amd/csrc/unet.cpp
@@ -5,6 +5,7 @@
 #include <map>
 #include <memory>
 
+#include "gn_finalize.h"
 #include "unet_internal.h"
 
 using namespace sisic;
@@ -338,7 +339,7 @@
         }
     }
 
-    int gn(const Buf* x, const Buf* skip, const NormW& n) {
+    int gn(const Buf* x, const Buf* skip, const NormW& n, GnFinJob* defer = nullptr, bool* deferred = nullptr) {
         gsc = u->gn_scale; gsh = u->gn_shift; gmr = nullptr; gnorm = &n;
         if (!tr && !skip && x->fin_norm == static_cast<const void*>(&n)) {
             gsc = x->fin_scale; gsh = x->fin_shift;
@@ -351,10 +352,16 @@
             SISIC_TRY(pool_get(u, (size_t)B * u->cfg.norm_groups * 2, &gmr));
             tr->grads_of_bufs.push_back(gsc); tr->grads_of_bufs.push_back(gsh); tr->grads_of_bufs.push_back(gmr);
         }
-        if (x->stats && (!skip || skip->stats))
+        if (x->stats && (!skip || skip->stats)) {
+            if (defer && !tr) {
+                *deferred = true;
+                return make_gn_fin_job(defer, x->stats, x->C, x->slots, skip ? skip->stats : nullptr, skip ? skip->C : 0,
+                                       skip ? skip->slots : 0, B, u->cfg.norm_groups, u->cfg.norm_eps, n.gamma, n.beta, gsc, gsh);
+            }
             return launch_gn_finalize(u->ctx, x->stats, x->C, x->slots, skip ? skip->stats : nullptr, skip ? skip->C : 0,
                                       skip ? skip->slots : 0, B, x->H * x->W, u->cfg.norm_groups, u->cfg.norm_eps,
                                       n.gamma, n.beta, gsc, gsh, s, gmr);
+        }
         return launch_gn_stats(u->ctx, x->p, x->C, skip ? skip->p : nullptr, skip ? skip->C : 0, B, x->H * x->W,
                                u->cfg.norm_groups, u->cfg.norm_eps, n.gamma, n.beta, gsc, gsh, s, gmr);
     }
@@ -362,7 +369,8 @@
     int conv(const ConvW& c, const float* in0, int c0, const float* in1, int c1, int H, int W, int stride, int ups,
              bool gn_prologue, bool silu, const float* chan_bias, const float* residual, float* out,
              Buf* normed_later = nullptr, Buf* xb = nullptr, Buf* skipb = nullptr, Buf* resb = nullptr, Buf* outb = nullptr,
-             const AttnW* qkv_of = nullptr, const NormW* next_norm = nullptr) {
+             const AttnW* qkv_of = nullptr, const NormW* next_norm = nullptr, const GnFinJob* rider = nullptr,
+             bool* carried = nullptr) {
         sisic_conv_args a{};
         a.in0 = in0; a.c0 = c0; a.in1 = in1; a.c1 = c1;
         a.B = B; a.Hin = H; a.Win = W; a.upsample = ups; a.ksize = c.k; a.stride = stride;
@@ -403,7 +411,7 @@
             op.residual = resb; op.out = outb; op.out_ptr = out;
             tr->tape.push_back(op);
         }
-        return launch_conv2d(u->ctx, a, s);
+        return launch_conv2d(u->ctx, a, s, rider, carried);
     }
 
     int resnet(const ResnetW& r, const Buf* x, const Buf* skip, Buf** out, const NormW* next_norm = nullptr) {
@@ -411,14 +419,27 @@
         const int H = x->H, W = x->W;
         const int c1 = skip ? skip->C : 0;
         SISIC_REQUIRE(x->C + c1 == r.cin, "unet: resnet expects %d input channels, got %d", r.cin, x->C + c1);
-        SISIC_TRY(gn(x, skip, r.norm1));
+        GnFinJob fin{};
+        bool deferred = false;
+        SISIC_TRY(gn(x, skip, r.norm1, (u->gn_rider && !tr && r.shortcut.k) ? &fin : nullptr, &deferred));
+        Buf* sc = nullptr;
+        if (deferred) {
+            bool carried = false;
+            sc = make(r.cout, H, W, &rc); SISIC_TRY(rc);
+            SISIC_TRY(conv(r.shortcut, x->p, x->C, skip ? skip->p : nullptr, c1, H, W, 1, 0, false, false, nullptr,
+                           nullptr, sc->p, nullptr, const_cast<Buf*>(x), const_cast<Buf*>(skip), nullptr, sc, nullptr, nullptr,
+                           &fin, &carried));
+            if (!carried) SISIC_TRY(launch_gn_finalize_job(u->ctx, fin, s));
+        }
         Buf* h = make(r.cout, H, W, &rc); SISIC_TRY(rc);
         SISIC_TRY(conv(r.conv1, x->p, x->C, skip ? skip->p : nullptr, c1, H, W, 1, 0, true, true,
                        tproj + r.temb_off, nullptr, h->p, h, const_cast<Buf*>(x), const_cast<Buf*>(skip), nullptr, h, nullptr, &r.norm2));
         const float* residual = x->p;
         Buf* resb = const_cast<Buf*>(x);
-        Buf* sc = nullptr;
-        if (r.shortcut.k) {
+        if (sc) {
+            residual = sc->p;
+            resb = sc;
+        } else if (r.shortcut.k) {
             sc = make(r.cout, H, W, &rc); SISIC_TRY(rc);
             SISIC_TRY(conv(r.shortcut, x->p, x->C, skip ? skip->p : nullptr, c1, H, W, 1, 0, false, false, nullptr,
                            nullptr, sc->p, nullptr, const_cast<Buf*>(x), const_cast<Buf*>(skip), nullptr, sc));
@@ -627,6 +648,7 @@
     u->freqs.assign(cfg->freqs, cfg->freqs + cfg->n_freqs);
     if (const char* e = std::getenv("SISIC_WINOGRAD")) u->use_winograd = std::atoi(e) != 0;
     if (const char* e = std::getenv("SISIC_FUSED_GN")) u->fuse_gn = std::atoi(e) != 0;
+    if (const char* e = std::getenv("SISIC_GN_RIDER")) u->gn_rider = std::atoi(e) != 0;
     if (const char* e = std::getenv("SISIC_GRAPH")) u->graph_mode = std::atoi(e) != 0 ? 1 : 0;
     u->cfg.freqs = nullptr;
     const int rc = describe(u);
diff --git a/synt_isic_amd/csrc/unet_internal.h b/synt_isic_amd/csrc/unet_internal.h
--- a/synt_isic_amd/csrc/unet_internal.h
+++ b/synt_isic_amd/csrc/unet_internal.h
@@ -179,6 +179,7 @@
     bool latency_mode = false;
     bool use_winograd = true;
     bool fuse_gn = true;
+    bool gn_rider = true;
     float* eps_buf = nullptr;
     size_t eps_floats = 0;
     std::unique_ptr<sisic::TrainState> train;
diff --git a/synt_isic_amd/ops.py b/synt_isic_amd/ops.py
--- a/synt_isic_amd/ops.py
+++ b/synt_isic_amd/ops.py
@@ -131,6 +131,37 @@
     return scale, shift
 
 
+def conv2d_gn_rider(x: torch.Tensor, w_packed: torch.Tensor, cout: int, ksize: int, stats: torch.Tensor, hw: int,
+                    gamma: torch.Tensor, beta: torch.Tensor, groups: int, eps: float, *, stats2: Optional[torch.Tensor] = None,
+                    bias=None, x2=None, gn_scale=None, gn_shift=None, gn_silu=False, tile_cfg=0, w_winograd=None,
+                    scale: Optional[torch.Tensor] = None, shift: Optional[torch.Tensor] = None):
+    lib = _lib.load()
+    B, c0, H, W = x.shape
+    c1 = 0 if x2 is None else x2.shape[1]
+    out = torch.empty((B, cout, H, W), dtype=torch.float32, device=x.device)
+    a = ConvArgs()
+    a.in0 = _ptr(x, "x"); a.in1 = _ptr(x2, "x2"); a.c0 = c0; a.c1 = c1
+    a.B = B; a.Hin = H; a.Win = W
+    a.upsample = 0; a.ksize = ksize; a.stride = 1
+    a.w_packed = _ptr(w_packed, "w_packed"); a.bias = _ptr(bias, "bias"); a.Cout = cout
+    a.gn_scale = _ptr(gn_scale, "gn_scale"); a.gn_shift = _ptr(gn_shift, "gn_shift"); a.gn_silu = int(gn_silu)
+    a.out = out.data_ptr(); a.tile_cfg = tile_cfg
+    a.w_winograd = _ptr(w_winograd, "w_winograd")
+    Bs, s0, slots0, _ = stats.shape
+    s1, slots1 = (0, 0) if stats2 is None else (stats2.shape[1], stats2.shape[2])
+    if scale is None:
+        scale = torch.empty((Bs, s0 + s1), dtype=torch.float32, device=stats.device)
+    if shift is None:
+        shift = torch.empty((Bs, s0 + s1), dtype=torch.float32, device=stats.device)
+    if tuple(scale.shape) != (Bs, s0 + s1) or tuple(shift.shape) != (Bs, s0 + s1):
+        raise ValueError(f"scale / shift must be {(Bs, s0 + s1)} tensors")
+    carried = C.c_int(0)
+    check(lib.sisic_conv2d_gn_rider(context(x.device), C.byref(a), _ptr(stats, "stats"), s0, slots0, _ptr(stats2, "stats2"),
+                                    s1, slots1, Bs, hw, groups, float(eps), _ptr(gamma, "gamma"), _ptr(beta, "beta"),
+                                    _ptr(scale, "scale"), _ptr(shift, "shift"), C.byref(carried), _stream(x.device)))
+    return out, scale, shift, carried.value
+
+
 def groupnorm_stats(x: torch.Tensor, gamma: torch.Tensor, beta: torch.Tensor, groups: int, eps: float,
                     x2: Optional[torch.Tensor] = None):
     lib = _lib.load()
```

After: 12.69, median of 6. +1.1%, better.
